# Spijkervet/Context-Aware-Sequential-Recommendation

Hardware: NVIDIA B200
Metric: train_seqs_per_sec (higher is better)
Workload: dtype f32

## Files before the change

### context-aware-sequential-recommendation_b200/_lib.py

```python
from __future__ import annotations

import ctypes as C
import os

_HERE = os.path.dirname(os.path.abspath(__file__))
LIB_PATH = os.path.join(_HERE, "csrc", "libcast_b200.so")

P, L, I, F, U64, SZ = C.c_void_p, C.c_long, C.c_int, C.c_float, C.c_ulonglong, C.c_size_t

SIGNATURES = {
    "cast_version": (I, []),
    "cast_last_error_string": (C.c_char_p, []),
    "cast_launch_count": (U64, []),
    "cast_crc32c": (C.c_uint, [P, SZ, C.c_uint]),
    "cast_embed_fwd": (I, [P, P, I, I, L, I, F, P, P, F, U64, P, I, P, P, P]),
    "cast_mask_dropout": (I, [P, P, F, U64, P, I, L, I, P, P, P]),
    "cast_concat_dropout_fwd": (I, [P, I, I, L, I, F, I, F, I, U64, P, P, P]),
    "cast_concat_dropout_bwd": (I, [P, I, I, L, I, F, I, F, I, U64, P, P, P]),
    "cast_dropout_keep": (I, [F, U64, P, I, L, P, P]),
    "cast_add": (I, [P, P, P, L, P]),
    "cast_relu_bwd": (I, [P, P, F, P, L, P]),
    "cast_layernorm_fwd": (I, [P, P, P, L, I, F, P, P, P, P, P, P]),
    "cast_layernorm_bwd_workspace_bytes": (SZ, [L, I]),
    "cast_layernorm_bwd": (I, [P, P, P, P, P, L, I, P, P, P, P, P, SZ, P]),
    "cast_gemm_set_backend": (I, [I]),
    "cast_gemm_tensor_status": (I, [P, P]),
    "cast_gemm_workspace_bytes": (SZ, [L, I, L, I]),
    "cast_gemm": (I, [P, L, L, P, L, L, P, L, L, I, L, P, I, F, U64, P, I, P, L, F, P, L, P, I, P, SZ, P]),
    "cast_fused_supported": (I, [I]),
    "cast_ln_qkv_fwd": (I, [P, P, P, P, P, P, P, P, P, L, I, F, P, P, P, P, P, P, P, P, P]),
    "cast_ln_ffn_fwd": (I, [P, P, P, P, P, P, P, P, F, U64, P, I, I, L, I, F, P, P, P, P, P, P]),
    "cast_rowk_supported": (I, [I]),
    "cast_rowk_image_bytes": (SZ, [I]),
    "cast_rowk_presplit": (I, [P, I, I, P, SZ, P]),
    "cast_rowk_ln_qkv_fwd": (I, [P, P, P, P, P, P, P, L, I, F, P, P, P, P, P, P, P, P, P]),
    "cast_rowk_ln_ffn_fwd": (I, [P, P, P, P, P, P, P, F, U64, P, I, I, L, I, F, P, P, P, P, P, P]),
    "cast_rowk_status": (I, [P]),
    "cast_rowk_set_grid": (I, [I]),
    "cast_rowk_set_trace": (I, [P]),
    "cast_block_bwd_workspace_bytes": (SZ, [L, I]),
    "cast_ffn_bwd": (I, [P, P, P, P, P, P, P, P, P, P, F, U64, P, I, L, I, P, P, P, SZ, P]),
    "cast_qkv_bwd": (I, [P, P, P, P, P, P, P, P, P, P, P, P, L, I, P, P, P, SZ, P]),
    "cast_qkv_bwd_embed": (I, [P, P, P, P, P, P, P, P, P, P, P, P, L, I, P, F, U64, P, I, P, P, P, SZ, P]),
    "cast_colsum_workspace_bytes": (SZ, [L, L]),
    "cast_colsum": (I, [P, L, L, L, P, P, SZ, P]),
    "cast_attn_set_chunk": (I, [I]),
    "cast_set_pdl": (I, [I]),
    "cast_attn_set_kg": (I, [I]),
    "cast_fused_set_backend": (I, [I]),
    "cast_block_bwd_parts": (I, [L, I]),
    "cast_reduce_partials_batch": (I, [I, P, P, P, P, P, P]),
    "cast_layernorm_bwd_parts": (I, [L]),
    "cast_logits_loss_parts": (I, [L]),
    "cast_sampler_create": (P, [I, I, P, P, P, P, P, P, I, C.c_uint, P, I]),
    "cast_sampler_next": (I, [P, I, P, P, P, P, P, P, P, P]),
    "cast_sampler_next_raw": (I, [P, I, P, P, P, P, P]),
    "cast_sampler_destroy": (None, [P]),
    "cast_time_features": (I, [P, P, P, I, I, P, I, P, P, P, P]),
    "cast_lnf_loss_parts": (I, [L]),
    "cast_lnf_loss_workspace_bytes": (SZ, [L, I]),
    "cast_lnf_loss": (I, [P, P, P, F, P, I, I, L, P, P, P, P, P, P, P, P, P, SZ, P]),
    "cast_attn_fwd": (I, [P, L, P, L, P, L, P, P, P, I, I, I, I, F, U64, P, I, P, P, P, P, P, P]),
    "cast_attn_bwd": (I, [P, L, P, L, P, L, P, P, P, P, P, P, P, I, I, I, I, F, U64, P, I, P, L, P, L, P, L, P, P, P, SZ,
                      P]),
    "cast_attn_bwd_workspace_bytes": (SZ, [I, I, I]),
    "cast_logits_loss_workspace_bytes": (SZ, [L]),
    "cast_logits_loss": (I, [P, P, I, I, L, P, P, P, P, P, P, P, P, P, SZ, P]),
    "cast_scatter_workspace_bytes": (SZ, [L, I, I]),
    "cast_scatter_partial_bytes": (SZ, [L, I, I]),
    "cast_scatter_rows": (I, [P, I, L, P, P, P, I, I, P, P, SZ, P, SZ, P]),
    "cast_scatter_sort": (I, [P, I, L, I, P, SZ, P]),
    "cast_scatter_apply": (I, [I, L, P, P, P, I, I, P, P, SZ, P, SZ, I, P]),
    "cast_adam_init_state": (I, [P, F, F, P]),
    "cast_adam_tf_step": (I, [P, P, P, P, L, F, F, F, F, P, F, L, L, P, P]),
    "cast_adam_tf_range": (I, [P, P, P, P, L, F, F, F, F, P, F, L, L, P, I, P]),
    "cast_adam_tf_step_peers": (I, [P, P, I, P, P, P, L, L, F, F, F, F, F, L, L, P, P]),
    "cast_score_rank_cand": (I, [P, L, P, I, I, L, P, I, P, P, P, P]),
    "cast_score_rank_full_workspace_bytes": (SZ, [L, I, I]),
    "cast_score_rank_full": (I, [P, L, P, I, I, L, P, P, P, P, I, P, P, P, P, SZ, P]),
    "cast_embed_fwd_sharded": (I, [P, P, I, I, I, L, I, F, P, P, F, U64, P, I, P, P, P]),
    "cast_logits_loss_sharded": (I, [P, P, I, I, I, L, P, P, P, P, P, P, P, P, P, SZ, P]),
    "cast_score_rank_cand_sharded": (I, [P, L, P, I, I, I, L, P, I, P, P, P, P]),
    "cast_scatter_set_chunk": (I, [I]),
    "cast_scatter_sort_sharded": (I, [P, I, L, I, I, I, P, SZ, P]),
    "cast_scatter_sorted_offsets": (I, [L, I, I, P, P]),
    "cast_scatter_apply_range": (I, [I, L, P, P, P, I, P, P, P, C.c_uint, C.c_uint, P, SZ, I, P]),
    "cast_scatter_stage_bytes": (SZ, [L, I, I]),
    "cast_scatter_pull_range": (I, [I, L, P, P, P, I, P, P, P, C.c_uint, C.c_uint, P, SZ, P, SZ, I, P]),
    "cast_peer_alloc": (I, [SZ, P, P]),
    "cast_peer_free": (I, [P]),
    "cast_peer_open": (I, [P, P]),
    "cast_peer_close": (I, [P]),
    "cast_peer_barrier": (I, [P, I, I, P, P]),
    "cast_peer_reduce": (I, [P, I, L, P, P]),
    "cast_score_rank_full_status": (I, [P, L, I, P, P]),
    "cast_topk_full_workspace_bytes": (SZ, [L, I, I, I]),
    "cast_topk_full": (I, [P, L, P, I, I, L, I, P, P, I, P, P, P, P, SZ, P]),
    "cast_topk_full_status": (I, [P, L, I, I, I, P, P]),
}


class CastError(RuntimeError):
    pass


def bind(lib: C.CDLL) -> C.CDLL:
    for name, (res, args) in SIGNATURES.items():
        try:
            fn = getattr(lib, name)
        except AttributeError as e:
            raise CastError(f"{name} is not exported by {getattr(lib, '_name', lib)}") from e
        fn.restype = res
        fn.argtypes = args
    return lib


_LIB = None


def load_library(path: str | None = None) -> C.CDLL:
    global _LIB
    if _LIB is not None and path is None:
        return _LIB
    p = path or LIB_PATH
    if not os.path.isfile(p):
        raise CastError(
            f"CUDA extension not found at {p}. Build it with `python -c 'import __graft_entry__ as g; g.build()'` "
            "(nvcc, sm_100a). This package has no CPU / PyTorch fallback.")
    lib = bind(C.CDLL(p))
    if os.environ.get("CAST_ATTN_CHUNK"):
        check(lib, lib.cast_attn_set_chunk(int(os.environ["CAST_ATTN_CHUNK"])), "cast_attn_set_chunk")
    if os.environ.get("CAST_PDL"):
        check(lib, lib.cast_set_pdl(int(os.environ["CAST_PDL"])), "cast_set_pdl")
    if os.environ.get("CAST_ATTN_KG"):
        check(lib, lib.cast_attn_set_kg(int(os.environ["CAST_ATTN_KG"])), "cast_attn_set_kg")
    if os.environ.get("CAST_FUSED_BACKEND"):
        check(lib, lib.cast_fused_set_backend(int(os.environ["CAST_FUSED_BACKEND"])), "cast_fused_set_backend")
    if path is None:
        _LIB = lib
    return lib


def check(lib: C.CDLL, rc: int, what: str = ""):
    if rc != 0:
        msg = lib.cast_last_error_string()
        raise CastError(f"{what} failed with code {rc}: {msg.decode() if msg else ''}")
```

### context-aware-sequential-recommendation_b200/csrc/row_umma.cu

```cuda
#include "cast_rt.cuh"
#include "mma_tf32.cuh"
#include "umma.cuh"

namespace cast {

constexpr int RU_ROWS = 128;
constexpr int RU_ROW_THREADS = 512;
constexpr int RU_THREADS = RU_ROW_THREADS + 32;
constexpr int RU_PA = RU_ROWS * 16 + 16;
constexpr int RU_NIMG = 9;
constexpr size_t RU_SMEM_MAX = 232448;

struct RuShape {
  int H, KS, SL, NP;
  int img1, img2;
  int dense;
};

__host__ __device__ inline RuShape ru_shape(int H) {
  RuShape s;
  s.H = H;
  s.KS = (H + 7) / 8;
  s.SL = 2 * s.KS;
  s.NP = (H + 15) / 16 * 16;
  s.img1 = 2 * s.SL * (s.NP * 16 + 16);
  s.img2 = 2 * s.SL * (2 * s.NP * 16 + 16);
  s.dense = (RU_ROWS * H * 4 + 15) & ~15;
  return s;
}

__host__ __device__ inline size_t ru_img_offset(const RuShape& s, int which) {
  size_t off = 0;
  for (int i = 0; i < which; ++i) off += (i == 1) ? s.img2 : s.img1;
  return off;
}
__host__ __device__ inline size_t ru_img_block_bytes(const RuShape& s) { return ru_img_offset(s, RU_NIMG); }

struct RuPresplitArgs {
  const float* w[16][5];
};

__global__ void __launch_bounds__(256) ru_presplit_kernel(RuPresplitArgs a, int H, unsigned char* __restrict__ images) {
  const RuShape s = ru_shape(H);
  const int blk = blockIdx.z, which = blockIdx.y;
  unsigned char* img = images + (size_t)blk * ru_img_block_bytes(s) + ru_img_offset(s, which);
  const int rows = (which == 1) ? 2 * s.NP : s.NP;
  const int pitch = rows * 16 + 16;
  const int half = s.SL * pitch;
  const int KP = 4 * s.SL;
  const bool transposed = which < 4;
  const int idx = blockIdx.x * (int)blockDim.x + threadIdx.x;
  if (idx >= rows * KP) return;
  int n, k;
  if (transposed) { k = idx / rows; n = idx - k * rows; } else { n = idx / KP; k = idx - n * KP; }
  const float* W;
  int nn = n;
  switch (which) {
    case 0: case 4: W = a.w[blk][0]; break;
    case 1: W = a.w[blk][n < s.NP ? 1 : 2]; nn = n < s.NP ? n : n - s.NP; break;
    case 2: case 7: W = a.w[blk][3]; break;
    case 3: case 8: W = a.w[blk][4]; break;
    case 5: W = a.w[blk][1]; break;
    default: W = a.w[blk][2]; break;
  }
  float v = 0.f;
  if (nn < H && k < H) v = transposed ? W[k * H + nn] : W[nn * H + k];
  unsigned hi, lo;
  tf32_split(v, hi, lo);
  const int off = (k >> 2) * pitch + n * 16 + (k & 3) * 4;
  *reinterpret_cast<unsigned*>(img + off) = hi;
  *reinterpret_cast<unsigned*>(img + half + off) = lo;
}


#ifndef CAST_EMU
__device__ __forceinline__ void ru_cp_async16(float* dst, const float* src, int bytes) {
  const unsigned d = (unsigned)__cvta_generic_to_shared(dst);
  asm volatile("cp.async.cg.shared.global [%0], [%1], 16, %2;" ::"r"(d), "l"(src), "r"(bytes) : "memory");
}
#else
inline void ru_cp_async16(float* dst, const float* src, int bytes) {
  for (int i = 0; i < 4; ++i) dst[i] = (4 * i < bytes) ? src[i] : 0.f;
}
#endif

__device__ __forceinline__ void ru_row_sync() { umma::named_sync(1, RU_ROW_THREADS); }

__device__ __forceinline__ void ru_tile_load_async(float* __restrict__ tile, const float* __restrict__ src, long nvalid,
                                                   int ntotal) {
  const int t = threadIdx.x;
  if ((reinterpret_cast<uintptr_t>(src) & 15) == 0) {
    for (int i = 4 * t; i < ntotal; i += 4 * RU_ROW_THREADS) {
      long left = (nvalid - i) * 4;
      const int bytes = left >= 16 ? 16 : (left > 0 ? (int)left : 0);
      ru_cp_async16(tile + i, bytes > 0 ? src + i : src, bytes);
    }
  } else {
    for (int i = t; i < ntotal; i += RU_ROW_THREADS) tile[i] = i < nvalid ? src[i] : 0.f;
  }
  cp_async_commit();
}

__device__ __forceinline__ void ru_tile_store(float* __restrict__ dst, const float* __restrict__ tile, long nvalid) {
  const int t = threadIdx.x;
  if ((reinterpret_cast<uintptr_t>(dst) & 15) == 0) {
    const int n4 = (int)(nvalid >> 2);
    for (int i = t; i < n4; i += RU_ROW_THREADS)
      reinterpret_cast<float4*>(dst)[i] = reinterpret_cast<const float4*>(tile)[i];
    for (int i = 4 * n4 + t; i < nvalid; i += RU_ROW_THREADS) dst[i] = tile[i];
  } else {
    for (int i = t; i < nvalid; i += RU_ROW_THREADS) dst[i] = tile[i];
  }
}

__device__ __forceinline__ void ru_row_load(const float* __restrict__ tile, int r, int c0, int H, float (&x)[16]) {
  const float* p = tile + r * H + c0;
  if ((H & 1) == 0) {
#pragma unroll
    for (int i = 0; i < 16; i += 2) {
      if (c0 + i < H) {
        const float2 v = *reinterpret_cast<const float2*>(p + i);
        x[i] = v.x;
        x[i + 1] = v.y;
      } else {
        x[i] = x[i + 1] = 0.f;
      }
    }
  } else {
#pragma unroll
    for (int i = 0; i < 16; ++i) x[i] = (c0 + i < H) ? p[i] : 0.f;
  }
}

__device__ __forceinline__ void ru_row_store(float* __restrict__ tile, int r, int c0, int H, const float (&x)[16]) {
  float* p = tile + r * H + c0;
  if ((H & 1) == 0) {
#pragma unroll
    for (int i = 0; i < 16; i += 2)
      if (c0 + i < H) *reinterpret_cast<float2*>(p + i) = make_float2(x[i], x[i + 1]);
  } else {
#pragma unroll
    for (int i = 0; i < 16; ++i)
      if (c0 + i < H) p[i] = x[i];
  }
}

__device__ __forceinline__ void ru_stage(unsigned char* __restrict__ hi, unsigned char* __restrict__ lo, int r, int qd,
                                         int SL, const float (&x)[16]) {
#pragma unroll
  for (int i = 0; i < 4; ++i) {
    const int s = 4 * qd + i;
    if (s < SL) {
      uint4 h, l;
      tf32_split(x[4 * i + 0], h.x, l.x);
      tf32_split(x[4 * i + 1], h.y, l.y);
      tf32_split(x[4 * i + 2], h.z, l.z);
      tf32_split(x[4 * i + 3], h.w, l.w);
      *reinterpret_cast<uint4*>(hi + s * RU_PA + r * 16) = h;
      *reinterpret_cast<uint4*>(lo + s * RU_PA + r * 16) = l;
    }
  }
}

__device__ __forceinline__ void ru_operand_ready(uint64_t* bar) {
  umma::fence_smem_to_async();
  umma::fence_before_sync();
  __syncwarp();
  if ((threadIdx.x & 31) == 0) umma::mbar_arrive(bar);
}

__device__ __forceinline__ void ru_issue(uint32_t tmem_d, uint32_t a_hi, uint32_t a_lo, uint32_t b_hi, uint32_t b_lo,
                                         uint32_t b_pitch, int KS, uint32_t idesc, uint32_t accumulate) {
  uint64_t dah = umma::smem_desc(a_hi, RU_PA, 128), dal = umma::smem_desc(a_lo, RU_PA, 128);
  uint64_t dbh = umma::smem_desc(b_hi, b_pitch, 128), dbl = umma::smem_desc(b_lo, b_pitch, 128);
  for (int ks = 0; ks < KS; ++ks) {
    umma::mma_tf32(tmem_d, dal, dbh, idesc, (ks > 0) ? 1u : accumulate);
    umma::mma_tf32(tmem_d, dah, dbl, idesc, 1u);
    umma::mma_tf32(tmem_d, dah, dbh, idesc, 1u);
    dah = umma::desc_advance(dah, 2 * RU_PA);
    dal = umma::desc_advance(dal, 2 * RU_PA);
    dbh = umma::desc_advance(dbh, 2 * b_pitch);
    dbl = umma::desc_advance(dbl, 2 * b_pitch);
  }
}

__device__ long long* g_rowk_trace = nullptr;
#ifndef CAST_EMU
#define RU_STAMP(slot, k)                                                                      \
  if (trace && threadIdx.x == 0 && (slot) < 4) trace[((long)blockIdx.x * 4 + (slot)) * 16 + (k)] = clock64()
#else
#define RU_STAMP(slot, k)
#endif

__device__ int g_rowk_timeout = 0;
__device__ __forceinline__ void ru_wait(uint64_t* bar, uint32_t parity) {
  if (!umma::mbar_wait(bar, parity, 1u << 22)) g_rowk_timeout = 1;
}

struct RuRange {
  long lo, hi;
  int ntiles;
};
__device__ __forceinline__ RuRange ru_range(long N, long rpc) {
  RuRange g;
  g.lo = (long)blockIdx.x * rpc;
  g.hi = g.lo + rpc < N ? g.lo + rpc : N;
  g.ntiles = g.hi > g.lo ? (int)((g.hi - g.lo + RU_ROWS - 1) / RU_ROWS) : 0;
  return g;
}

struct RuLn {
  float mean, rstd, xsum;
};
template <class F>
__device__ __forceinline__ RuLn ru_layernorm(const float (&x)[16], float (&y)[16], const float* __restrict__ gamma,
                                             const float* __restrict__ beta, float eps, int r, int qd, int c0, int H,
                                             float* __restrict__ red, F&& between) {
  float sp = 0.f;
#pragma unroll
  for (int i = 0; i < 16; ++i) sp += x[i];
  red[r * 4 + qd] = sp;
  ru_row_sync();
  between();
  RuLn o;
  {
    const float4 p = *reinterpret_cast<const float4*>(red + r * 4);
    o.xsum = (p.x + p.y) + (p.z + p.w);
  }
  o.mean = o.xsum / (float)H;
  float qp = 0.f;
#pragma unroll
  for (int i = 0; i < 16; ++i) {
    const float d = (c0 + i < H) ? x[i] - o.mean : 0.f;
    y[i] = d;
    qp += d * d;
  }
  red[512 + r * 4 + qd] = qp;
  ru_row_sync();
  {
    const float4 p = *reinterpret_cast<const float4*>(red + 512 + r * 4);
    o.rstd = 1.0f / sqrtf(((p.x + p.y) + (p.z + p.w)) / (float)H + eps);
  }
  float yp = 0.f;
#pragma unroll
  for (int i = 0; i < 16; i += 4) {
    const float4 g = *reinterpret_cast<const float4*>(gamma + c0 + i);
    const float4 b = *reinterpret_cast<const float4*>(beta + c0 + i);
    y[i + 0] = (c0 + i + 0 < H) ? g.x * (y[i + 0] * o.rstd) + b.x : 0.f;
    y[i + 1] = (c0 + i + 1 < H) ? g.y * (y[i + 1] * o.rstd) + b.y : 0.f;
    y[i + 2] = (c0 + i + 2 < H) ? g.z * (y[i + 2] * o.rstd) + b.z : 0.f;
    y[i + 3] = (c0 + i + 3 < H) ? g.w * (y[i + 3] * o.rstd) + b.w : 0.f;
    yp += (y[i] + y[i + 1]) + (y[i + 2] + y[i + 3]);
  }
  red[1024 + r * 4 + qd] = yp;
  return o;
}

struct RuLnQkvArgs {
  const float *x, *gamma, *beta, *bq, *bk, *bv;
  const unsigned char* img;
  float eps;
  float *qn, *Q, *K, *V, *mean, *rstd, *kmask, *qmask;
  long N, rpc;
  int H;
};

__global__ void __launch_bounds__(RU_THREADS, 1) ru_ln_qkv_fwd_kernel(RuLnQkvArgs a) {
  CAST_DYN_SMEM(unsigned char, sm);
  __shared__ __align__(8) uint64_t bars[5];
  __shared__ uint32_t tmem_slot;
  const RuShape s = ru_shape(a.H);
  const int H = a.H;
  unsigned char* wq = sm;
  unsigned char* wkv = wq + s.img1;
  unsigned char* a_hi = wkv + s.img2;
  unsigned char* a_lo = a_hi + s.SL * RU_PA;
  float* tin = reinterpret_cast<float*>(a_lo + s.SL * RU_PA);
  float* out0 = tin + s.dense / 4;
  float* out1 = out0 + s.dense / 4;
  float* vec = out1 + s.dense / 4;
  float* red = vec + 5 * 64;
  const int t = threadIdx.x, warp = t >> 5, r = t & 127, qd = (t >> 7) & 3, c0 = 16 * qd;
  const bool have_cols = c0 < H;
  long long* trace = g_rowk_trace;
  RU_STAMP(0, 0);

  if (t == 0) {
    umma::mbar_init(&bars[0], 1);
    umma::mbar_init(&bars[1], RU_ROW_THREADS / 32);
    umma::mbar_init(&bars[2], RU_ROW_THREADS / 32);
    umma::mbar_init(&bars[3], 1);
    umma::mbar_init(&bars[4], 1);
  }
  if (warp == 0) umma::tmem_alloc(&tmem_slot, 256);
  for (int i = t; i < 5 * 64; i += RU_THREADS) {
    const int which = i >> 6, c = i & 63;
    const float* src = which == 0 ? a.gamma : which == 1 ? a.beta : which == 2 ? a.bq : which == 3 ? a.bk : a.bv;
    vec[i] = c < H ? src[c] : 0.f;
  }
  umma::fence_before_sync();
  __syncthreads();
  umma::fence_after_sync();
  const uint32_t tmem = tmem_slot;
  const RuRange rg = ru_range(a.N, a.rpc);
  const uint32_t idesc_q = umma::idesc_tf32(128, s.NP), idesc_kv = umma::idesc_tf32(128, 2 * s.NP);

  if (warp == RU_ROW_THREADS / 32) {
    if ((t & 31) == 0 && rg.ntiles > 0) {
      umma::mbar_arrive_expect_tx(&bars[0], (uint32_t)(s.img1 + s.img2));
      umma::bulk_g2s(wq, a.img + ru_img_offset(s, 0), (uint32_t)s.img1, &bars[0]);
      umma::bulk_g2s(wkv, a.img + ru_img_offset(s, 1), (uint32_t)s.img2, &bars[0]);
      cast_pdl_wait();
      ru_wait(&bars[0], 0);
      for (int it = 0; it < rg.ntiles; ++it) {
        const uint32_t par = (uint32_t)(it & 1);
        ru_wait(&bars[1], par);
        umma::fence_after_sync();
        ru_issue(tmem + (uint32_t)s.NP, umma::smem_u32(a_hi), umma::smem_u32(a_lo), umma::smem_u32(wkv),
                 umma::smem_u32(wkv + s.img2 / 2), (uint32_t)(2 * s.NP * 16 + 16), s.KS, idesc_kv, 0u);
        umma::mma_commit(&bars[3]);
        ru_wait(&bars[2], par);
        umma::fence_after_sync();
        ru_issue(tmem, umma::smem_u32(a_hi), umma::smem_u32(a_lo), umma::smem_u32(wq), umma::smem_u32(wq + s.img1 / 2),
                 (uint32_t)(s.NP * 16 + 16), s.KS, idesc_q, 0u);
        umma::mma_commit(&bars[4]);
      }
    }
    __syncwarp();
  } else {
    const int ntot = RU_ROWS * H;
    auto rows_of = [&](int it) {
      const long left = rg.hi - (rg.lo + (long)it * RU_ROWS);
      return left < RU_ROWS ? left : (long)RU_ROWS;
    };
    cast_pdl_wait();
    if (rg.ntiles > 0) ru_tile_load_async(tin, a.x + rg.lo * H, rows_of(0) * H, ntot);
    const uint32_t lane_base = ((uint32_t)(warp & 3) * 32u) << 16;
    for (int it = 0; it < rg.ntiles; ++it) {
      const long row0 = rg.lo + (long)it * RU_ROWS, row = row0 + r;
      const long vrows = rows_of(it), nvalid = vrows * H;
      const uint32_t par = (uint32_t)(it & 1);
      cp_async_wait<0>();
      ru_row_sync();
      RU_STAMP(it, 1);
      float x[16], q[16];
      ru_row_load(tin, r, c0, H, x);
      ru_stage(a_hi, a_lo, r, qd, s.SL, x);
      ru_operand_ready(&bars[1]);
      RU_STAMP(it, 2);
      const RuLn ln = ru_layernorm(x, q, vec, vec + 64, a.eps, r, qd, c0, H, red, [&]() {
        if (it + 1 < rg.ntiles) ru_tile_load_async(tin, a.x + (row0 + RU_ROWS) * H, rows_of(it + 1) * H, ntot);
      });
      RU_STAMP(it, 3);
      ru_row_store(out0, r, c0, H, q);
      ru_wait(&bars[3], par);
      umma::fence_after_sync();
      RU_STAMP(it, 4);
      ru_stage(a_hi, a_lo, r, qd, s.SL, q);
      ru_operand_ready(&bars[2]);
      ru_row_sync();
      RU_STAMP(it, 5);
      if (qd == 0 && row < rg.hi) {
        const float4 p = *reinterpret_cast<const float4*>(red + 1024 + r * 4);
        const float ysum = (p.x + p.y) + (p.z + p.w);
        a.mean[row] = ln.mean;
        a.rstd[row] = ln.rstd;
        if (a.kmask) a.kmask[row] = ln.xsum != 0.f ? 1.f : 0.f;
        if (a.qmask) a.qmask[row] = ysum != 0.f ? 1.f : 0.f;
      }
      ru_tile_store(a.qn + row0 * H, out0, nvalid);
      float v[16];
      if (have_cols) {
        umma::tmem_ld16(tmem + lane_base + (uint32_t)(s.NP + c0), v);
#pragma unroll
        for (int i = 0; i < 16; ++i) v[i] += vec[3 * 64 + c0 + i];
        ru_row_store(out1, r, c0, H, v);
      }
      ru_row_sync();
      RU_STAMP(it, 6);
      ru_tile_store(a.K + row0 * H, out1, nvalid);
      if (have_cols) {
        umma::tmem_ld16(tmem + lane_base + (uint32_t)(2 * s.NP + c0), v);
#pragma unroll
        for (int i = 0; i < 16; ++i) v[i] += vec[4 * 64 + c0 + i];
        ru_row_store(out0, r, c0, H, v);
      }
      ru_row_sync();
      RU_STAMP(it, 7);
      ru_tile_store(a.V + row0 * H, out0, nvalid);
      ru_wait(&bars[4], par);
      umma::fence_after_sync();
      RU_STAMP(it, 8);
      if (have_cols) {
        umma::tmem_ld16(tmem + lane_base + (uint32_t)c0, v);
#pragma unroll
        for (int i = 0; i < 16; ++i) v[i] += vec[2 * 64 + c0 + i];
        ru_row_store(out1, r, c0, H, v);
      }
      umma::fence_before_sync();
      ru_row_sync();
      ru_tile_store(a.Q + row0 * H, out1, nvalid);
      RU_STAMP(it, 9);
    }
    cp_async_wait<0>();
  }
  umma::fence_before_sync();
  __syncthreads();
  if (warp == 0) umma::tmem_free(tmem, 256);
}

struct RuLnFfnArgs {
  const float *y, *gamma, *beta, *b1, *b2;
  const unsigned char* img;
  const int* ids;
  float eps, rate;
  unsigned long long seed;
  const unsigned long long* step;
  int site_h, site_o;
  float *zn, *h1d, *xout, *mean, *rstd;
  long N, rpc;
  int H;
};

__global__ void __launch_bounds__(RU_THREADS, 1) ru_ln_ffn_fwd_kernel(RuLnFfnArgs a) {
  CAST_DYN_SMEM(unsigned char, sm);
  __shared__ __align__(8) uint64_t bars[5];
  __shared__ uint32_t tmem_slot;
  const RuShape s = ru_shape(a.H);
  const int H = a.H;
  unsigned char* w1 = sm;
  unsigned char* w2 = w1 + s.img1;
  unsigned char* a_hi = w2 + s.img1;
  unsigned char* a_lo = a_hi + s.SL * RU_PA;
  float* tin = reinterpret_cast<float*>(a_lo + s.SL * RU_PA);
  float* out0 = tin + s.dense / 4;
  float* out1 = out0 + s.dense / 4;
  float* vec = out1 + s.dense / 4;
  float* red = vec + 4 * 64;
  const int t = threadIdx.x, warp = t >> 5, r = t & 127, qd = (t >> 7) & 3, c0 = 16 * qd;
  const bool have_cols = c0 < H;
  long long* trace = g_rowk_trace;
  RU_STAMP(0, 0);

  if (t == 0) {
    umma::mbar_init(&bars[0], 1);
    umma::mbar_init(&bars[1], RU_ROW_THREADS / 32);
    umma::mbar_init(&bars[2], RU_ROW_THREADS / 32);
    umma::mbar_init(&bars[3], 1);
    umma::mbar_init(&bars[4], 1);
  }
  if (warp == 0) umma::tmem_alloc(&tmem_slot, 128);
  for (int i = t; i < 4 * 64; i += RU_THREADS) {
    const int which = i >> 6, c = i & 63;
    const float* src = which == 0 ? a.gamma : which == 1 ? a.beta : which == 2 ? a.b1 : a.b2;
    vec[i] = c < H ? src[c] : 0.f;
  }
  umma::fence_before_sync();
  __syncthreads();
  umma::fence_after_sync();
  const uint32_t tmem = tmem_slot;
  const RuRange rg = ru_range(a.N, a.rpc);
  const uint32_t idesc = umma::idesc_tf32(128, s.NP);
  const uint32_t wpitch = (uint32_t)(s.NP * 16 + 16);

  if (warp == RU_ROW_THREADS / 32) {
    if ((t & 31) == 0 && rg.ntiles > 0) {
      umma::mbar_arrive_expect_tx(&bars[0], (uint32_t)(2 * s.img1));
      umma::bulk_g2s(w1, a.img + ru_img_offset(s, 2), (uint32_t)(2 * s.img1), &bars[0]);
      cast_pdl_wait();
      ru_wait(&bars[0], 0);
      for (int it = 0; it < rg.ntiles; ++it) {
        const uint32_t par = (uint32_t)(it & 1);
        ru_wait(&bars[1], par);
        umma::fence_after_sync();
        ru_issue(tmem, umma::smem_u32(a_hi), umma::smem_u32(a_lo), umma::smem_u32(w1), umma::smem_u32(w1 + s.img1 / 2),
                 wpitch, s.KS, idesc, 0u);
        umma::mma_commit(&bars[3]);
        ru_wait(&bars[2], par);
        umma::fence_after_sync();
        ru_issue(tmem + (uint32_t)s.NP, umma::smem_u32(a_hi), umma::smem_u32(a_lo), umma::smem_u32(w2),
                 umma::smem_u32(w2 + s.img1 / 2), wpitch, s.KS, idesc, 0u);
        umma::mma_commit(&bars[4]);
      }
    }
    __syncwarp();
  } else {
    const int ntot = RU_ROWS * H;
    auto rows_of = [&](int it) {
      const long left = rg.hi - (rg.lo + (long)it * RU_ROWS);
      return left < RU_ROWS ? left : (long)RU_ROWS;
    };
    cast_pdl_wait();
    if (rg.ntiles > 0) ru_tile_load_async(tin, a.y + rg.lo * H, rows_of(0) * H, ntot);
    const uint32_t lane_base = ((uint32_t)(warp & 3) * 32u) << 16;
    const Drop dh = make_drop(a.rate, a.seed, a.step, a.site_h);
    const Drop dout = make_drop(a.rate, a.seed, a.step, a.site_o);
    for (int it = 0; it < rg.ntiles; ++it) {
      const long row0 = rg.lo + (long)it * RU_ROWS, row = row0 + r;
      const long vrows = rows_of(it), nvalid = vrows * H;
      const uint32_t par = (uint32_t)(it & 1);
      const float m = (row < rg.hi && a.ids) ? (a.ids[row] != 0 ? 1.f : 0.f) : 1.f;
      cp_async_wait<0>();
      ru_row_sync();
      RU_STAMP(it, 1);
      float x[16], zn[16];
      ru_row_load(tin, r, c0, H, x);
      const RuLn ln = ru_layernorm(x, zn, vec, vec + 64, a.eps, r, qd, c0, H, red, [&]() {
        if (it + 1 < rg.ntiles) ru_tile_load_async(tin, a.y + (row0 + RU_ROWS) * H, rows_of(it + 1) * H, ntot);
      });
      RU_STAMP(it, 2);
      ru_stage(a_hi, a_lo, r, qd, s.SL, zn);
      ru_operand_ready(&bars[1]);
      ru_row_store(out0, r, c0, H, zn);
      if (qd == 0 && row < rg.hi) {
        a.mean[row] = ln.mean;
        a.rstd[row] = ln.rstd;
      }
      ru_row_sync();
      RU_STAMP(it, 3);
      ru_tile_store(a.zn + row0 * H, out0, nvalid);
      ru_wait(&bars[3], par);
      umma::fence_after_sync();
      RU_STAMP(it, 4);
      float v[16];
      const unsigned long long fi0 = (unsigned long long)(row * H + c0);
      const bool fi_even = (fi0 & 1ull) == 0ull;
      if (have_cols) {
        umma::tmem_ld16(tmem + lane_base + (uint32_t)c0, v);
        float dm[16];
        if (fi_even) {
#pragma unroll
          for (int i = 0; i < 16; i += 2) drop_mul2_even(dh, fi0 + i, dm[i], dm[i + 1]);
        } else {
#pragma unroll
          for (int i = 0; i < 16; i += 2) drop_mul2(dh, fi0 + i, dm[i], dm[i + 1]);
        }
#pragma unroll
        for (int i = 0; i < 16; ++i) {
          const int c = c0 + i;
          v[i] = (c < H) ? fmaxf(v[i] + vec[2 * 64 + c], 0.f) * dm[i] : 0.f;
        }
        ru_row_store(out1, r, c0, H, v);
      } else {
#pragma unroll
        for (int i = 0; i < 16; ++i) v[i] = 0.f;
      }
      ru_stage(a_hi, a_lo, r, qd, s.SL, v);
      ru_operand_ready(&bars[2]);
      ru_row_sync();
      RU_STAMP(it, 5);
      ru_tile_store(a.h1d + row0 * H, out1, nvalid);
      ru_wait(&bars[4], par);
      umma::fence_after_sync();
      RU_STAMP(it, 6);
      if (have_cols) {
        umma::tmem_ld16(tmem + lane_base + (uint32_t)(s.NP + c0), v);
        float dm[16];
        if (fi_even) {
#pragma unroll
          for (int i = 0; i < 16; i += 2) drop_mul2_even(dout, fi0 + i, dm[i], dm[i + 1]);
        } else {
#pragma unroll
          for (int i = 0; i < 16; i += 2) drop_mul2(dout, fi0 + i, dm[i], dm[i + 1]);
        }
#pragma unroll
        for (int i = 0; i < 16; ++i) v[i] = ((v[i] + vec[3 * 64 + ((c0 + i) & 63)]) * dm[i] + zn[i]) * m;
        ru_row_store(out0, r, c0, H, v);
      }
      umma::fence_before_sync();
      ru_row_sync();
      ru_tile_store(a.xout + row0 * H, out0, nvalid);
      RU_STAMP(it, 7);
    }
    cp_async_wait<0>();
  }
  umma::fence_before_sync();
  __syncthreads();
  if (warp == 0) umma::tmem_free(tmem, 128);
}

static size_t ru_ln_qkv_smem(const RuShape& s) {
  return (size_t)s.img1 + s.img2 + 2 * (size_t)s.SL * RU_PA + 3 * (size_t)s.dense + (5 * 64 + 3 * 512) * sizeof(float);
}
static size_t ru_ln_ffn_smem(const RuShape& s) {
  return 2 * (size_t)s.img1 + 2 * (size_t)s.SL * RU_PA + 3 * (size_t)s.dense + (4 * 64 + 3 * 512) * sizeof(float);
}

constexpr int RU_NUM_SMS = 148;

}

using namespace cast;

#define CAST_RU_SMEM(kernel, bytes)                                                            \
  {                                                                                            \
    static size_t configured = 48 * 1024;                                                      \
    if ((bytes) > configured) {                                                                \
      cudaFuncSetAttribute(kernel, cudaFuncAttributeMaxDynamicSharedMemorySize, (int)(bytes)); \
      configured = (bytes);                                                                    \
    }                                                                                          \
  }

static int g_rowk_max_ctas = RU_NUM_SMS;
extern "C" int cast_rowk_set_grid(int max_ctas) {
  if (max_ctas < 1) return set_error(CAST_ERR_BAD_ARG, "rowk_set_grid");
  g_rowk_max_ctas = max_ctas < RU_NUM_SMS ? max_ctas : RU_NUM_SMS;
  return CAST_OK;
}

extern "C" int cast_rowk_supported(int H) {
  if (H < 8 || H > 64) return 0;
  const RuShape s = ru_shape(H);
  return ru_ln_qkv_smem(s) <= RU_SMEM_MAX && ru_ln_ffn_smem(s) <= RU_SMEM_MAX;
}

extern "C" size_t cast_rowk_image_bytes(int H) {
  if (H <= 0 || H > 64) return 0;
  return ru_img_block_bytes(ru_shape(H));
}

extern "C" int cast_rowk_presplit(const float* const* weights, int nblocks, int H, void* images, size_t image_bytes,
                                  void* stream) {
  if (!weights || !images || nblocks <= 0) return set_error(CAST_ERR_BAD_ARG, "rowk_presplit");
  if (!cast_rowk_supported(H)) return set_error(CAST_ERR_UNSUPPORTED, "rowk_presplit: hidden_units not supported");
  const size_t per = cast_rowk_image_bytes(H);
  if (image_bytes < per * (size_t)nblocks) return set_error(CAST_ERR_WORKSPACE, "rowk_presplit: image buffer too small");
  for (int b0 = 0; b0 < nblocks; b0 += 16) {
    const int nb = nblocks - b0 < 16 ? nblocks - b0 : 16;
    RuPresplitArgs a;
    for (int b = 0; b < 16; ++b)
      for (int j = 0; j < 5; ++j) a.w[b][j] = b < nb ? weights[(size_t)(b0 + b) * 5 + j] : nullptr;
    for (int b = 0; b < nb; ++b)
      for (int j = 0; j < 5; ++j)
        if (!a.w[b][j]) return set_error(CAST_ERR_BAD_ARG, "rowk_presplit: null weight pointer");
    const RuShape s = ru_shape(H);
    CAST_LAUNCH(ru_presplit_kernel, dim3((unsigned)cdiv(2L * s.NP * 4 * s.SL, 256), RU_NIMG, (unsigned)nb), dim3(256), 0,
                (cudaStream_t)stream, a, H, static_cast<unsigned char*>(images) + (size_t)b0 * per);
  }
  return check_launch("rowk_presplit");
}

extern "C" int cast_rowk_ln_qkv_fwd(const float* x, const float* gamma, const float* beta, const float* bq,
                                    const float* bk, const float* bv, const void* images, long N, int H, float eps,
                                    float* qn, float* Q, float* K, float* V, float* mean, float* rstd, float* kmask,
                                    float* qmask, void* stream) {
  if (!x || !gamma || !beta || !bq || !bk || !bv || !images || !qn || !Q || !K || !V || !mean || !rstd || N <= 0)
    return set_error(CAST_ERR_BAD_ARG, "rowk_ln_qkv_fwd");
  if (!cast_rowk_supported(H)) return set_error(CAST_ERR_UNSUPPORTED, "rowk_ln_qkv_fwd: hidden_units not supported");
  const RuShape s = ru_shape(H);
  const long ntiles = cdiv(N, RU_ROWS);
  const int grid = (int)(ntiles < g_rowk_max_ctas ? ntiles : g_rowk_max_ctas);
  const long rpc = cdiv(cdiv(N, grid), 4) * 4;
  RuLnQkvArgs a{x, gamma, beta, bq, bk, bv, static_cast<const unsigned char*>(images), eps, qn, Q, K, V, mean, rstd,
                kmask, qmask, N, rpc, H};
  const size_t smem = ru_ln_qkv_smem(s);
  CAST_RU_SMEM(ru_ln_qkv_fwd_kernel, smem)
  CAST_LAUNCH_DEP(ru_ln_qkv_fwd_kernel, dim3(grid), dim3(RU_THREADS), smem, (cudaStream_t)stream, a);
  return check_launch("rowk_ln_qkv_fwd");
}

extern "C" int cast_rowk_ln_ffn_fwd(const float* y, const float* gamma, const float* beta, const float* b1,
                                    const float* b2, const void* images, const int* ids, float drop_rate,
                                    unsigned long long seed, const unsigned long long* step, int site_hidden,
                                    int site_out, long N, int H, float eps, float* zn, float* h1d, float* xout,
                                    float* mean, float* rstd, void* stream) {
  if (!y || !gamma || !beta || !b1 || !b2 || !images || !zn || !h1d || !xout || !mean || !rstd || N <= 0)
    return set_error(CAST_ERR_BAD_ARG, "rowk_ln_ffn_fwd");
  if (!cast_rowk_supported(H)) return set_error(CAST_ERR_UNSUPPORTED, "rowk_ln_ffn_fwd: hidden_units not supported");
  if (drop_rate < 0.f || drop_rate >= 1.f) return set_error(CAST_ERR_BAD_ARG, "rowk_ln_ffn_fwd: drop_rate");
  const RuShape s = ru_shape(H);
  const long ntiles = cdiv(N, RU_ROWS);
  const int grid = (int)(ntiles < g_rowk_max_ctas ? ntiles : g_rowk_max_ctas);
  const long rpc = cdiv(cdiv(N, grid), 4) * 4;
  RuLnFfnArgs a{y, gamma, beta, b1, b2, static_cast<const unsigned char*>(images), ids, eps, drop_rate, seed, step,
                site_hidden, site_out, zn, h1d, xout, mean, rstd, N, rpc, H};
  const size_t smem = ru_ln_ffn_smem(s);
  CAST_RU_SMEM(ru_ln_ffn_fwd_kernel, smem)
  CAST_LAUNCH_DEP(ru_ln_ffn_fwd_kernel, dim3(grid), dim3(RU_THREADS), smem, (cudaStream_t)stream, a);
  return check_launch("rowk_ln_ffn_fwd");
}

extern "C" int cast_rowk_set_trace(void* device_buffer) {
#ifndef CAST_EMU
  long long* p = static_cast<long long*>(device_buffer);
  if (cudaMemcpyToSymbol(g_rowk_trace, &p, sizeof(p)) != cudaSuccess) return set_error(CAST_ERR_CUDA, "rowk_set_trace");
#endif
  return CAST_OK;
}

extern "C" int cast_rowk_status(int* timed_out) {
  if (!timed_out) return set_error(CAST_ERR_BAD_ARG, "rowk_status");
#ifdef CAST_EMU
  *timed_out = g_rowk_timeout;
  g_rowk_timeout = 0;
#else
  int v = 0, zero = 0;
  if (cudaDeviceSynchronize() != cudaSuccess) return set_error(CAST_ERR_CUDA, "rowk_status: device error");
  cudaMemcpyFromSymbol(&v, g_rowk_timeout, sizeof(int));
  cudaMemcpyToSymbol(g_rowk_timeout, &zero, sizeof(int));
  *timed_out = v;
#endif
  return CAST_OK;
}
```

### context-aware-sequential-recommendation_b200/engine.py

```python
from __future__ import annotations

import ctypes as C
import math
import os
from types import SimpleNamespace
from typing import Dict, List, Optional

import numpy as np
import torch

from . import _lib

TOWER_ID = {"main": 0, "time": 1, "hours": 2, "days": 3}
SITE_EMBED, SITE_CONCAT_A, SITE_CONCAT_B = 9000, 9001, 9002
MODELS = ["cast_1", "cast_2", "cast_3", "cast_4", "cast_5", "cast_6", "cast_7", "cast_8", "cast_9", "sasrec",
          "sasrec_static"]
TABLE_ROWS = {"hours_emb": 25, "days_emb": 8}


def block_site(tower: str, block: int, k: int) -> int:
    return 1000 * TOWER_ID[tower] + 10 * block + k


def sinusoid_table(dim: int, length: int) -> np.ndarray:
    pos = np.arange(length, dtype=np.float64)[:, None]
    i = np.arange(dim, dtype=np.float64)[None, :]
    v = (pos / np.power(10000.0, 2.0 * i / dim)).reshape(-1)
    v[::2] = np.sin(v[::2])
    v[1::2] = np.cos(v[1::2])
    return v.reshape(length, dim).astype(np.float32)


def model_plan(model: str, args) -> SimpleNamespace:
    m = model.lower()
    if m not in MODELS:
        raise ValueError(f"provide model from {MODELS}")
    L, Lc = args.num_blocks, getattr(args, "num_context_blocks", 2)
    p = SimpleNamespace(model=m, towers={}, tables=["item_emb"], learned_pos=m in ("sasrec", "cast_9"))
    if m in ("cast_1", "cast_2", "cast_3", "cast_4", "cast_5", "cast_6"):
        p.towers["time"] = L
        p.tables.append("time_emb")
    if m in ("cast_3", "cast_4", "cast_5", "cast_6", "cast_7", "cast_8", "cast_9"):
        p.tables += ["hours_emb", "days_emb"]
    if m == "cast_8":
        p.towers["hours"] = L
        p.towers["days"] = L
    if m == "cast_9":
        p.towers["hours"] = Lc
        p.towers["days"] = Lc
        p.towers["time"] = Lc
        p.tables.append("time_emb")
    p.towers["main"] = L
    p.embed = {"sasrec": (False, True, True), "sasrec_static": (False, True, True), "cast_1": (True, True, True),
               "cast_2": (False, False, True), "cast_3": (True, False, True), "cast_4": (False, False, True),
               "cast_5": (True, False, False), "cast_6": (False, False, False), "cast_7": (False, False, True),
               "cast_8": (False, False, True), "cast_9": (False, False, False)}[m]
    p.merge = {"cast_2": (["seq", "time"], 2, False, "pre", False),
               "cast_3": (["seq", "hours", "days"], 3, False, "pre", False),
               "cast_4": (["seq", "time", "hours", "days"], 2, True, "pre", False),
               "cast_5": (["seq", "hours", "days"], 3, False, "post", False),
               "cast_6": (["seq", "time", "hours", "days"], 2, True, "post", False),
               "cast_7": (["seq", "hours", "days"], 3, False, "pre", False),
               "cast_8": (["seq", "hours", "days"], 3, False, "pre", False),
               "cast_9": (["seq", "time", "hours", "days"], 4, False, "pre", True)}.get(m)
    p.attn_tower = "time" if m in ("cast_1", "cast_2", "cast_3", "cast_4", "cast_5", "cast_6") else "main"
    return p


def shard_rows(itemnum: int, world: int) -> int:
    return (itemnum + 1 + world - 1) // world + 1


def param_shapes(plan, args, itemnum: int, item_rows: Optional[int] = None):
    H, T = args.hidden_units, args.maxlen
    out = []
    rows = {"item_emb": itemnum + 1, "time_emb": args.max_bins + 1, **TABLE_ROWS}
    for t in plan.tables:
        if t == "item_emb" and item_rows is not None:
            out.append((t, (item_rows, H), rows[t], H))
            continue
        out.append((t, (rows[t], H), rows[t], H))
    if plan.learned_pos:
        out.append(("pos_emb", (T, H), T, H))
    n_tables = len(out)
    for tower, nb in plan.towers.items():
        for i in range(nb):
            pre = f"{tower}.{i}."
            out.append((pre + "ln1.beta", (H,), None, 0.0))
            out.append((pre + "ln1.gamma", (H,), None, 1.0))
            for d in ("q", "k", "v"):
                out.append((pre + d + ".w", (H, H), H, H))
                out.append((pre + d + ".b", (H,), None, 0.0))
            out.append((pre + "ln2.beta", (H,), None, 0.0))
            out.append((pre + "ln2.gamma", (H,), None, 1.0))
            for d in ("ffn1", "ffn2"):
                out.append((pre + d + ".w", (H, H), H, H))
                out.append((pre + d + ".b", (H,), None, 0.0))
        out.append((f"{tower}.lnf.beta", (H,), None, 0.0))
        out.append((f"{tower}.lnf.gamma", (H,), None, 1.0))
    if plan.merge:
        k = len(plan.merge[0]) * H
        out += [("mlp.0.w", (k, k), k, k), ("mlp.0.b", (k,), None, 0.0), ("mlp.1.w", (k, H), k, H),
                ("mlp.1.b", (H,), None, 0.0)]
    return out, n_tables


class Engine:

    def __init__(self, model: str, usernum: int, itemnum: int, args, device=None, lib=None, seed: Optional[int] = None,
                 item_shard: Optional[tuple] = None, alloc=None):
        self.lib = lib if lib is not None else _lib.load_library()
        self.timing = None
        self.use_fused = True
        if device is None:
            if not torch.cuda.is_available():
                raise _lib.CastError("no CUDA device: this package has no CPU fallback")
            device = torch.device("cuda", torch.cuda.current_device())
        self.device = torch.device(device)
        self.args = args
        self.plan = model_plan(model, args)
        self.usernum, self.itemnum = usernum, itemnum
        self.H, self.T, self.h = args.hidden_units, args.maxlen, args.num_heads
        if self.H % self.h:
            raise ValueError("hidden_units must be divisible by num_heads")
        self.rate = float(args.dropout_rate)
        self.lr = float(args.lr)
        self.l2 = float(getattr(args, "l2_emb", 0.0))
        self.seed = int(seed if seed is not None else (getattr(args, "seed", 0) or 0))
        self.beta1, self.beta2, self.eps = 0.9, 0.98, 1e-8
        self.item_shard = tuple(item_shard) if item_shard is not None and item_shard[1] > 1 else None
        self.V_items = itemnum + 1
        self.shard_R = shard_rows(itemnum, self.item_shard[1]) if self.item_shard else None
        self.alloc = alloc
        self.arena = None
        if self.item_shard is not None and alloc is None:
            from . import dist as _dist
            self.arena = _dist.PeerArena(self.lib, self.device)
            self.alloc = self.arena.alloc
        shapes, n_tables = param_shapes(self.plan, args, itemnum, self.shard_R)
        self.shapes = shapes
        total = sum(int(np.prod(s)) for _, s, _, _ in shapes)
        f32 = dict(dtype=torch.float32, device=self.device)
        self.w = self._peer_zeros(total, torch.float32)
        self.gbuf = torch.zeros(total + 4, **f32)
        self.g = self.gbuf[:total]
        self.sums = self.gbuf[total:]
        self.m = torch.zeros(total, **f32)
        self.v = torch.zeros(total, **f32)
        self.P: Dict[str, torch.Tensor] = {}
        self.G: Dict[str, torch.Tensor] = {}
        self.offsets: Dict[str, int] = {}
        off = 0
        for idx, (name, shape, _, _) in enumerate(shapes):
            n = int(np.prod(shape))
            self.P[name] = self.w[off:off + n].view(*shape)
            self.G[name] = self.g[off:off + n].view(*shape)
            self.offsets[name] = off
            off += n
            if idx == n_tables - 1:
                self.l2_hi = off
        self.n_params = total
        self.adam_state = torch.zeros(2, dtype=torch.int64, device=self.device)
        self.step_ptr = self.adam_state.data_ptr() + 8
        self.sinus = torch.from_numpy(sinusoid_table(self.H, self.T)).to(self.device)
        self.init_parameters(self.seed or 42)
        self._call(self.lib.cast_adam_init_state, self.adam_state.data_ptr(), self.beta1, self.beta2, self._stream())
        self._ctx: Dict[tuple, SimpleNamespace] = {}
        self.use_rowk = bool(self.lib.cast_rowk_supported(self.H))
        self.rowk_block: Dict[str, int] = {}
        if self.use_rowk:
            names = [f"{tower}.{i}." for tower, nb in self.plan.towers.items() for i in range(nb)]
            self.rowk_block = {n: j for j, n in enumerate(names)}
            self.rowk_img_bytes = int(self.lib.cast_rowk_image_bytes(self.H))
            self.rowk_img = torch.zeros(max(1, len(names)) * self.rowk_img_bytes, dtype=torch.uint8, device=self.device)
            ptrs = [self.P[n + w].data_ptr() for n in names for w in ("q.w", "k.w", "v.w", "ffn1.w", "ffn2.w")]
            self.rowk_wptrs = (C.c_void_p * len(ptrs))(*ptrs)
        self.world_size = 1
        self.grad_allreduce = None
        self.adam_g = self.gbuf
        self.exchange_capturable = False
        self.after_adam = None
        if self.device.type == "cuda":
            self.lib.cast_set_pdl(0 if os.environ.get("CAST_PDL", "1") == "0" else 1)
        self.fork_reduce = os.environ.get("CAST_FORK_REDUCE", "1") != "0"
        self.fuse_embed_bwd = os.environ.get("CAST_FUSE_EMBED_BWD", "1") != "0"
        self.before_backward = None
        self.peer_adam = None
        self.shard_ptrs = None

    def _peer_zeros(self, numel, dtype):
        if self.alloc is not None and self.item_shard is not None:
            t = self.alloc(int(numel), dtype)
            t.zero_()
            return t
        return torch.zeros(int(numel), dtype=dtype, device=self.device)

    def _stream(self):
        if self.device.type == "cuda":
            return torch.cuda.current_stream(self.device).cuda_stream
        return None

    def _call(self, fn, *a):
        if self.timing is not None:
            e0, e1 = torch.cuda.Event(enable_timing=True), torch.cuda.Event(enable_timing=True)
            e0.record()
            rc = fn(*a)
            e1.record()
            self.timing.append((fn.__name__, a, e0, e1))
        else:
            rc = fn(*a)
        if rc != 0:
            _lib.check(self.lib, rc, fn.__name__)

    @staticmethod
    def _p(t):
        return None if t is None else t.data_ptr()

    def init_parameters(self, seed: int):
        gen = torch.Generator().manual_seed(seed)
        for name, shape, fan_in, fan_out in self.shapes:
            if fan_in is None:
                self.P[name].fill_(float(fan_out))
            else:
                limit = math.sqrt(6.0 / (fan_in + fan_out))
                if name == "item_emb" and self.item_shard is not None:
                    full = (torch.rand((self.V_items, shape[1]), generator=gen, dtype=torch.float64) * 2 - 1)
                    self.P[name].copy_(self.shard_of(full.mul(limit).float()).to(self.device))
                    continue
                vals = (torch.rand(shape, generator=gen, dtype=torch.float64) * 2 - 1).mul(limit).float()
                self.P[name].copy_(vals.to(self.device))
        self.m.zero_()
        self.v.zero_()

    def shard_of(self, full: torch.Tensor) -> torch.Tensor:
        rank, world = self.item_shard
        out = torch.zeros((self.shard_R,) + tuple(full.shape[1:]), dtype=full.dtype)
        mine = full[rank::world]
        off = 1 if rank else 0
        out[off:off + mine.shape[0]] = mine
        return out

    def rebind_gradients(self, gbuf: torch.Tensor):
        assert gbuf.numel() == self.gbuf.numel()
        local = self.adam_g is self.gbuf
        self.gbuf = gbuf
        self.g = gbuf[:self.n_params]
        self.sums = gbuf[self.n_params:]
        for name, shape, _, _ in self.shapes:
            off = self.offsets[name]
            self.G[name] = self.g[off:off + int(np.prod(shape))].view(*shape)
        if local:
            self.adam_g = gbuf
        for c in self._ctx.values():
            c.sums = self.sums

    def global_sums(self) -> torch.Tensor:
        return self.adam_g[self.n_params:]

    def load_parameters(self, params: Dict[str, "torch.Tensor | np.ndarray"]):
        for k, v in params.items():
            v = torch.as_tensor(np.asarray(v) if not torch.is_tensor(v) else v)
            if k == "item_emb" and self.item_shard is not None and v.shape[0] == self.V_items:
                v = self.shard_of(v)
            self.P[k].copy_(v.to(self.device))

    def state_step(self) -> int:
        return int(self.adam_state[1].item())

    def ctx(self, B: int) -> SimpleNamespace:
        key = (B, bool(self.use_fused))
        c = self._ctx.get(key)
        if c is not None:
            return c
        H, T, h, dev = self.H, self.T, self.h, self.device
        N = B * T
        lib = self.lib
        f = lambda *s: torch.empty(*s, dtype=torch.float32, device=dev)
        fp = (lambda *s: self._peer_zeros(int(np.prod(s)), torch.float32).view(*s)) if self.item_shard else f
        c = SimpleNamespace(B=B, N=N)
        c.keys3 = torch.zeros(3, N, dtype=torch.int32, device=dev)
        c.cids = torch.zeros(3, N, dtype=torch.int32, device=dev)
        c.tw = {}
        for tower, nb in self.plan.towers.items():
            blocks = []
            for _ in range(nb):
                b = SimpleNamespace()
                for nm in ("qn", "Q", "K", "V", "y", "zn", "h1d", "xout"):
                    setattr(b, nm, f(N, H))
                for nm in ("mu1", "rs1", "kmask", "qmask", "mu2", "rs2"):
                    setattr(b, nm, f(N))
                for nm in ("rmax", "rlinv", "rowD"):
                    setattr(b, nm, f(B * h * T))
                if self.use_fused and bool(self.lib.cast_fused_supported(H)):
                    nws = self.lib.cast_block_bwd_workspace_bytes(N, H) // 4 + 16
                    b.ws_ffn, b.ws_qkv = f(nws), f(nws)
                blocks.append(b)
            c.tw[tower] = SimpleNamespace(blocks=blocks, out=(fp if tower == "main" else f)(N, H), muf=f(N), rsf=f(N),
                                          dx_in=f(N, H), x_in=None)
        c.attn_ws = None
        if H // h <= 64 and 2 * B * h * T * T * 4 <= (2 << 30):
            c.attn_ws = torch.empty(self.lib.cast_attn_bwd_workspace_bytes(B, T, h) // 4, dtype=torch.float32, device=dev)
        c.x0 = f(N, H)
        c.emb = {t: f(N, H) for t in self.plan.tables if t != "item_emb"}
        c.demb = {t: f(N, H) for t in self.plan.tables if t != "item_emb"}
        if self.plan.merge:
            k = len(self.plan.merge[0])
            c.cat, c.mlp_h, c.mlp_out = f(N, k * H), f(N, k * H), fp(N, H)
            c.dcat, c.dmlp_h, c.dmlp_o = f(N, k * H), f(N, k * H), f(N, H)
            c.dsrc = {s: f(N, H) for s in self.plan.merge[0]}
        c.pos_logits, c.neg_logits, c.gpos, c.gneg = f(N), f(N), fp(N), fp(N)
        c.sums = self.sums
        c.dseq = f(N, H)
        c.t = [f(N, H) for _ in range(7)]
        c.g0 = fp(N, H)
        kmax = (len(self.plan.merge[0]) if self.plan.merge else 1) * H
        c.splits = int(max(1, min(296, N // 128)))
        ws = max(lib.cast_layernorm_bwd_workspace_bytes(N, H),
                 lib.cast_gemm_workspace_bytes(kmax, kmax, N, c.splits), lib.cast_gemm_workspace_bytes(N, kmax, kmax, 1),
                 lib.cast_colsum_workspace_bytes(N, kmax), lib.cast_colsum_workspace_bytes(B, T * H),
                 lib.cast_logits_loss_workspace_bytes(N), lib.cast_block_bwd_workspace_bytes(N, H))
        c.ws = torch.empty(ws // 4 + 16, dtype=torch.float32, device=dev)
        c.ws_bytes = ws
        vmax = max(self.P[t].shape[0] for t in self.plan.tables)
        if self.item_shard:
            vmax = max(vmax, self.item_shard[1] * self.shard_R)
        sws = lib.cast_scatter_workspace_bytes(N, 3, vmax)
        c.sws = self._peer_zeros(sws // 4 + 16, torch.int32) if self.item_shard else \
            torch.empty(sws // 4 + 16, dtype=torch.int32, device=dev)
        c.sws_bytes = sws
        c.peer = None
        spb = lib.cast_scatter_partial_bytes(N, 3, H)
        c.spart = torch.empty(spb // 4 + 16, dtype=torch.float32, device=dev)
        c.spart_bytes = spb
        c.attn = None
        c.graph = None
        self._ctx[key] = c
        return c

    def _gemm(self, A, sam, sak, Bm, sbk, sbn, Cm, ldc, M, N, K, c, bias=None, relu=0, rate=0.0, site=0, act=None,
              ld_act=0, act_scale=1.0, resid=None, ldr=0, row_ids=None, splits=1):
        self._call(self.lib.cast_gemm, A.data_ptr(), sam, sak, Bm.data_ptr(), sbk, sbn, Cm.data_ptr(), ldc, M, N, K,
                   self._p(bias), relu, rate, self.seed, self.step_ptr, site, self._p(act), ld_act, act_scale,
                   self._p(resid), ldr, self._p(row_ids), splits, c.ws.data_ptr(), c.ws_bytes, self._stream())

    def linear_fwd(self, c, X, W, b, Y, **kw):
        N, K = X.shape
        M = W.shape[1]
        self._gemm(X, K, 1, W, M, 1, Y, M, N, M, K, c, bias=b, **kw)

    def linear_dgrad(self, c, dY, W, dX, **kw):
        N, M = dY.shape
        K = W.shape[0]
        self._gemm(dY, M, 1, W, 1, M, dX, K, N, K, M, c, **kw)

    def linear_wgrad(self, c, X, dY, dW, db):
        N, K = X.shape
        M = dY.shape[1]
        self._gemm(X, 1, K, dY, M, 1, dW, M, K, M, N, c, splits=c.splits)
        if db is not None:
            self._call(self.lib.cast_colsum, dY.data_ptr(), N, M, M, db.data_ptr(), c.ws.data_ptr(), c.ws_bytes,
                       self._stream())

    def ln_fwd(self, x, pre, y, mu, rs, xnz=None, ynz=None):
        N = x.shape[0]
        self._call(self.lib.cast_layernorm_fwd, x.data_ptr(), self.P[pre + ".gamma"].data_ptr(),
                   self.P[pre + ".beta"].data_ptr(), N, self.H, 1e-8, y.data_ptr(), self._p(mu), self._p(rs),
                   self._p(xnz), self._p(ynz), self._stream())

    def ln_bwd(self, c, dy, x, mu, rs, pre, dx, dx_add=None):
        N = x.shape[0]
        self._call(self.lib.cast_layernorm_bwd, dy.data_ptr(), x.data_ptr(), mu.data_ptr(), rs.data_ptr(),
                   self.P[pre + ".gamma"].data_ptr(), N, self.H, self._p(dx_add), dx.data_ptr(),
                   self.G[pre + ".gamma"].data_ptr(), self.G[pre + ".beta"].data_ptr(), c.ws.data_ptr(), c.ws_bytes,
                   self._stream())

    def embed_fwd(self, ids, table, out, pos=None, add=None, rate=0.0, site=0, mask_ids=None):
        N = ids.numel()
        if self.item_shard is not None and table is self.P["item_emb"]:
            self._call(self.lib.cast_embed_fwd_sharded, ids.data_ptr(), self.shard_ptrs.data_ptr(), self.item_shard[1],
                       self.V_items, self.H, N, self.T, float(self.H ** 0.5), self._p(pos), self._p(add), rate,
                       self.seed, self.step_ptr, site, self._p(mask_ids), out.data_ptr(), self._stream())
            return
        self._call(self.lib.cast_embed_fwd, ids.data_ptr(), table.data_ptr(), table.shape[0], self.H, N, self.T,
                   float(self.H ** 0.5), self._p(pos), self._p(add), rate, self.seed, self.step_ptr, site,
                   self._p(mask_ids), out.data_ptr(), self._stream())

    def mask_dropout(self, x, ids, rate, site, out_m, out_md):
        N = x.shape[0]
        self._call(self.lib.cast_mask_dropout, x.data_ptr(), self._p(ids), rate, self.seed, self.step_ptr, site, N,
                   x.shape[1], self._p(out_m), self._p(out_md), self._stream())

    def scatter(self, c, keys, nsrc, rows, rowscale, scale, table_name):
        N = c.N
        V = self.P[table_name].shape[0]
        rows_a = (C.c_void_p * nsrc)(*[r.data_ptr() for r in rows])
        rs_a = (C.c_void_p * nsrc)(*[(r.data_ptr() if r is not None else None) for r in rowscale])
        sc_a = (C.c_float * nsrc)(*scale)
        if table_name == "item_emb" and self.item_shard is not None:
            if getattr(c, "presorted", False):
                torch.cuda.current_stream(self.device).wait_stream(c.side)
                c.presorted = False
            else:
                self._call(self.lib.cast_scatter_sort_sharded, keys.data_ptr(), nsrc, N, self.V_items,
                           self.item_shard[1], self.shard_R, c.sws.data_ptr(), c.sws_bytes, self._stream())
            if rows[0] is not c.g0:
                c.g0.copy_(rows[0])
            c.shard_src = (nsrc, [c.g0] + list(rows[1:]), list(rowscale), list(scale))
            return
        if table_name == "item_emb" and getattr(c, "presorted", False):
            torch.cuda.current_stream(self.device).wait_stream(c.side)
            c.presorted = False
            self._call(self.lib.cast_scatter_apply, nsrc, N, rows_a, rs_a, sc_a, V, self.H,
                       self.G[table_name].data_ptr(), c.sws.data_ptr(), c.sws_bytes, c.spart.data_ptr(),
                       c.spart_bytes, 0, self._stream())
            return
        self._call(self.lib.cast_scatter_rows, keys.data_ptr(), nsrc, N, rows_a, rs_a, sc_a, V, self.H,
                   self.G[table_name].data_ptr(), c.sws.data_ptr(), c.sws_bytes, c.spart.data_ptr(), c.spart_bytes,
                   self._stream())

    def tower_fwd(self, c, tower, x_in, ids, train, want_attn=False):
        tb = c.tw[tower]
        tb.x_in = x_in
        rate = self.rate if train else 0.0
        H, B, T, h = self.H, c.B, self.T, self.h
        x = x_in
        nb = len(tb.blocks)
        fused = self.use_fused and bool(self.lib.cast_fused_supported(H))
        rowk = self.rowk_active()
        if rowk and getattr(c, "presplit_pending", False):
            torch.cuda.current_stream(self.device).wait_stream(c.side2)
            c.presplit_pending = False
        P = self.P
        for i, b in enumerate(tb.blocks):
            pre = f"{tower}.{i}."
            if rowk:
                self._call(self.lib.cast_rowk_ln_qkv_fwd, x.data_ptr(), P[pre + "ln1.gamma"].data_ptr(),
                           P[pre + "ln1.beta"].data_ptr(), P[pre + "q.b"].data_ptr(), P[pre + "k.b"].data_ptr(),
                           P[pre + "v.b"].data_ptr(), self.rowk_image(pre), c.N, H, 1e-8, b.qn.data_ptr(),
                           b.Q.data_ptr(), b.K.data_ptr(), b.V.data_ptr(), b.mu1.data_ptr(), b.rs1.data_ptr(),
                           b.kmask.data_ptr(), b.qmask.data_ptr(), self._stream())
            elif fused:
                self._call(self.lib.cast_ln_qkv_fwd, x.data_ptr(), P[pre + "ln1.gamma"].data_ptr(),
                           P[pre + "ln1.beta"].data_ptr(), P[pre + "q.w"].data_ptr(), P[pre + "q.b"].data_ptr(),
                           P[pre + "k.w"].data_ptr(), P[pre + "k.b"].data_ptr(), P[pre + "v.w"].data_ptr(),
                           P[pre + "v.b"].data_ptr(), c.N, H, 1e-8, b.qn.data_ptr(), b.Q.data_ptr(), b.K.data_ptr(),
                           b.V.data_ptr(), b.mu1.data_ptr(), b.rs1.data_ptr(), b.kmask.data_ptr(),
                           b.qmask.data_ptr(), self._stream())
            else:
                self.ln_fwd(x, pre + "ln1", b.qn, b.mu1, b.rs1, b.kmask, b.qmask)
                self.linear_fwd(c, b.qn, self.P[pre + "q.w"], self.P[pre + "q.b"], b.Q)
                self.linear_fwd(c, x, self.P[pre + "k.w"], self.P[pre + "k.b"], b.K)
                self.linear_fwd(c, x, self.P[pre + "v.w"], self.P[pre + "v.b"], b.V)
            attn = None
            if want_attn and i == nb - 1:
                if c.attn is None or c.attn.shape[0] != h * B:
                    c.attn = torch.empty(h * B, T, T, dtype=torch.float32, device=self.device)
                attn = c.attn
            self._call(self.lib.cast_attn_fwd, b.Q.data_ptr(), H, b.K.data_ptr(), H, b.V.data_ptr(), H,
                       b.qn.data_ptr(), b.kmask.data_ptr(), b.qmask.data_ptr(), B, T, H, h, rate, self.seed,
                       self.step_ptr, block_site(tower, i, 1), ids.data_ptr(), b.y.data_ptr(), self._p(attn),
                       b.rmax.data_ptr(), b.rlinv.data_ptr(), self._stream())
            if rowk:
                self._call(self.lib.cast_rowk_ln_ffn_fwd, b.y.data_ptr(), P[pre + "ln2.gamma"].data_ptr(),
                           P[pre + "ln2.beta"].data_ptr(), P[pre + "ffn1.b"].data_ptr(), P[pre + "ffn2.b"].data_ptr(),
                           self.rowk_image(pre), ids.data_ptr(), rate, self.seed, self.step_ptr,
                           block_site(tower, i, 2), block_site(tower, i, 3), c.N, H, 1e-8, b.zn.data_ptr(),
                           b.h1d.data_ptr(), b.xout.data_ptr(), b.mu2.data_ptr(), b.rs2.data_ptr(), self._stream())
            elif fused:
                self._call(self.lib.cast_ln_ffn_fwd, b.y.data_ptr(), P[pre + "ln2.gamma"].data_ptr(),
                           P[pre + "ln2.beta"].data_ptr(), P[pre + "ffn1.w"].data_ptr(), P[pre + "ffn1.b"].data_ptr(),
                           P[pre + "ffn2.w"].data_ptr(), P[pre + "ffn2.b"].data_ptr(), ids.data_ptr(), rate,
                           self.seed, self.step_ptr, block_site(tower, i, 2), block_site(tower, i, 3), c.N, H, 1e-8,
                           b.zn.data_ptr(), b.h1d.data_ptr(), b.xout.data_ptr(), b.mu2.data_ptr(), b.rs2.data_ptr(),
                           self._stream())
            else:
                self.ln_fwd(b.y, pre + "ln2", b.zn, b.mu2, b.rs2)
                self.linear_fwd(c, b.zn, self.P[pre + "ffn1.w"], self.P[pre + "ffn1.b"], b.h1d, relu=1, rate=rate,
                                site=block_site(tower, i, 2))
                self.linear_fwd(c, b.h1d, self.P[pre + "ffn2.w"], self.P[pre + "ffn2.b"], b.xout, rate=rate,
                                site=block_site(tower, i, 3), resid=b.zn, ldr=H, row_ids=ids)
            x = b.xout
        if tower == "main" and train and getattr(c, "fuse_tail", False):
            tb.x_last = x
            return tb.out
        self.ln_fwd(x, tower + ".lnf", tb.out, tb.muf, tb.rsf)
        return tb.out

    def tower_bwd(self, c, tower, d_out, ids, embed_fx=None):
        tb = c.tw[tower]
        H, B, T, h = self.H, c.B, self.T, self.h
        rate = self.rate
        scale = 1.0 / (1.0 - rate) if rate > 0 else 1.0
        t = c.t
        nb = len(tb.blocks)
        x_last = tb.blocks[-1].xout if nb else tb.x_in
        fused = self.use_fused and bool(self.lib.cast_fused_supported(H))
        dx = t[0]
        if tower == "main" and getattr(c, "fuse_tail", False):
            pass
        elif fused:
            if getattr(tb, "ws_lnf", None) is None:
                nb_ = self.lib.cast_layernorm_bwd_workspace_bytes(c.N, H)
                tb.ws_lnf = torch.empty(nb_ // 4 + 16, dtype=torch.float32, device=self.device)
            self._call(self.lib.cast_layernorm_bwd, d_out.data_ptr(), x_last.data_ptr(), tb.muf.data_ptr(),
                       tb.rsf.data_ptr(), self.P[tower + ".lnf.gamma"].data_ptr(), c.N, H, None, dx.data_ptr(), None,
                       None, tb.ws_lnf.data_ptr(), tb.ws_lnf.numel() * 4, self._stream())
            parts = self.lib.cast_layernorm_bwd_parts(c.N)
            c.reduce_jobs.append((tb.ws_lnf.data_ptr(), parts, H, self.G[tower + ".lnf.gamma"], 2 * H))
            c.reduce_jobs.append((tb.ws_lnf.data_ptr() + 4 * H, parts, H, self.G[tower + ".lnf.beta"], 2 * H))
        else:
            self.ln_bwd(c, d_out, x_last, tb.muf, tb.rsf, tower + ".lnf", dx)
        for i in reversed(range(nb)):
            b = tb.blocks[i]
            pre = f"{tower}.{i}."
            x_i = tb.blocks[i - 1].xout if i > 0 else tb.x_in
            gm, gmd, dh, dzn, dy = t[1], t[2], t[3], t[4], t[5]
            if fused:
                P = self.P
                self._call(self.lib.cast_ffn_bwd, dx.data_ptr(), ids.data_ptr(), b.zn.data_ptr(), b.h1d.data_ptr(),
                           b.y.data_ptr(), b.mu2.data_ptr(), b.rs2.data_ptr(), P[pre + "ln2.gamma"].data_ptr(),
                           P[pre + "ffn1.w"].data_ptr(), P[pre + "ffn2.w"].data_ptr(), rate, self.seed, self.step_ptr,
                           block_site(tower, i, 3), c.N, H, dy.data_ptr(), None,
                           b.ws_ffn.data_ptr(), b.ws_ffn.numel() * 4, self._stream())
                cnt = 2 * H + 2 * (H * H + H)
                c.reduce_jobs.append((b.ws_ffn.data_ptr(), self.lib.cast_block_bwd_parts(c.N, 0), cnt,
                                      self.G[pre + "ln2.beta"], cnt))
                dQ, dK, dV = t[1], t[2], t[3]
                self._call(self.lib.cast_attn_bwd, b.Q.data_ptr(), H, b.K.data_ptr(), H, b.V.data_ptr(), H,
                           dy.data_ptr(), b.kmask.data_ptr(), b.qmask.data_ptr(), b.rmax.data_ptr(),
                           b.rlinv.data_ptr(), ids.data_ptr(), b.rowD.data_ptr(), B, T, H, h, rate, self.seed,
                           self.step_ptr,
                           block_site(tower, i, 1), dQ.data_ptr(), H, dK.data_ptr(), H, dV.data_ptr(), H,
                           b.y.data_ptr(), b.qn.data_ptr(), self._p(c.attn_ws),
                           c.attn_ws.numel() * 4 if c.attn_ws is not None else 0, self._stream())
                dst = tb.dx_in if i == 0 else t[0]
                if i == 0 and embed_fx is not None:
                    fx_ids, fx_rate, fx_site, dst = embed_fx
                    self._call(self.lib.cast_qkv_bwd_embed, dQ.data_ptr(), dK.data_ptr(), dV.data_ptr(),
                               dy.data_ptr(), x_i.data_ptr(), b.qn.data_ptr(), b.mu1.data_ptr(), b.rs1.data_ptr(),
                               P[pre + "ln1.gamma"].data_ptr(), P[pre + "q.w"].data_ptr(), P[pre + "k.w"].data_ptr(),
                               P[pre + "v.w"].data_ptr(), c.N, H, self._p(fx_ids), float(fx_rate), self.seed,
                               self.step_ptr, int(fx_site), dst.data_ptr(), None, b.ws_qkv.data_ptr(),
                               b.ws_qkv.numel() * 4, self._stream())
                else:
                    self._call(self.lib.cast_qkv_bwd, dQ.data_ptr(), dK.data_ptr(), dV.data_ptr(), dy.data_ptr(),
                               x_i.data_ptr(), b.qn.data_ptr(), b.mu1.data_ptr(), b.rs1.data_ptr(),
                               P[pre + "ln1.gamma"].data_ptr(), P[pre + "q.w"].data_ptr(), P[pre + "k.w"].data_ptr(),
                               P[pre + "v.w"].data_ptr(), c.N, H, dst.data_ptr(), None,
                               b.ws_qkv.data_ptr(), b.ws_qkv.numel() * 4, self._stream())
                cnt = 2 * H + 3 * (H * H + H)
                c.reduce_jobs.append((b.ws_qkv.data_ptr(), self.lib.cast_block_bwd_parts(c.N, 1), cnt,
                                      self.G[pre + "ln1.beta"], cnt))
                dx = dst
                continue
            self.mask_dropout(dx, ids, rate, block_site(tower, i, 3), gm, gmd)
            self.linear_wgrad(c, b.h1d, gmd, self.G[pre + "ffn2.w"], self.G[pre + "ffn2.b"])
            self.linear_dgrad(c, gmd, self.P[pre + "ffn2.w"], dh, act=b.h1d, ld_act=H, act_scale=scale)
            self.linear_wgrad(c, b.zn, dh, self.G[pre + "ffn1.w"], self.G[pre + "ffn1.b"])
            self.linear_dgrad(c, dh, self.P[pre + "ffn1.w"], dzn, resid=gm, ldr=H)
            self.ln_bwd(c, dzn, b.y, b.mu2, b.rs2, pre + "ln2", dy)
            dQ, dK, dV = t[1], t[2], t[3]
            self._call(self.lib.cast_attn_bwd, b.Q.data_ptr(), H, b.K.data_ptr(), H, b.V.data_ptr(), H,
                       dy.data_ptr(), b.kmask.data_ptr(), b.qmask.data_ptr(), b.rmax.data_ptr(), b.rlinv.data_ptr(),
                       ids.data_ptr(), b.rowD.data_ptr(), B, T, H, h, rate, self.seed, self.step_ptr,
                       block_site(tower, i, 1),
                       dQ.data_ptr(), H, dK.data_ptr(), H, dV.data_ptr(), H, b.y.data_ptr(), b.qn.data_ptr(),
                       self._p(c.attn_ws), c.attn_ws.numel() * 4 if c.attn_ws is not None else 0, self._stream())
            self.linear_wgrad(c, b.qn, dQ, self.G[pre + "q.w"], self.G[pre + "q.b"])
            self.linear_wgrad(c, x_i, dK, self.G[pre + "k.w"], self.G[pre + "k.b"])
            self.linear_wgrad(c, x_i, dV, self.G[pre + "v.w"], self.G[pre + "v.b"])
            dqn, dxk, dxkv = t[4], t[6], t[0]
            self.linear_dgrad(c, dQ, self.P[pre + "q.w"], dqn, resid=dy, ldr=H)
            self.linear_dgrad(c, dK, self.P[pre + "k.w"], dxk)
            self.linear_dgrad(c, dV, self.P[pre + "v.w"], dxkv, resid=dxk, ldr=H)
            dst = tb.dx_in if i == 0 else t[5]
            self.ln_bwd(c, dqn, x_i, b.mu1, b.rs1, pre + "ln1", dst, dx_add=dxkv)
            dx = dst
        if nb == 0:
            tb.dx_in.copy_(dx)
        return tb.dx_in

    def merge_fwd(self, c, srcs: Dict[str, torch.Tensor], ids, train):
        names, wa, second, _, mask_after = self.plan.merge
        k = len(names)
        rate = self.rate if train else 0.0
        ptrs = (C.c_void_p * k)(*[srcs[n].data_ptr() for n in names])
        if second:
            ra, sa, rb, sb = rate, SITE_CONCAT_A, rate, SITE_CONCAT_B
        else:
            wa, ra, sa, rb, sb = 0, 0.0, SITE_CONCAT_A, rate, SITE_CONCAT_A
        self._call(self.lib.cast_concat_dropout_fwd, ptrs, k, wa, c.N, self.H, ra, sa, rb, sb, self.seed,
                   self.step_ptr, c.cat.data_ptr(), self._stream())
        self.linear_fwd(c, c.cat, self.P["mlp.0.w"], self.P["mlp.0.b"], c.mlp_h, relu=1)
        self.linear_fwd(c, c.mlp_h, self.P["mlp.1.w"], self.P["mlp.1.b"], c.mlp_out, relu=1,
                        row_ids=ids if mask_after else None)
        return c.mlp_out

    def merge_bwd(self, c, d_out):
        names, wa, second, _, _ = self.plan.merge
        k = len(names)
        rate = self.rate
        n1 = c.N * self.H
        self._call(self.lib.cast_relu_bwd, d_out.data_ptr(), c.mlp_out.data_ptr(), 1.0, c.dmlp_o.data_ptr(), n1,
                   self._stream())
        self.linear_wgrad(c, c.mlp_h, c.dmlp_o, self.G["mlp.1.w"], self.G["mlp.1.b"])
        self.linear_dgrad(c, c.dmlp_o, self.P["mlp.1.w"], c.dmlp_h, act=c.mlp_h, ld_act=k * self.H, act_scale=1.0)
        self.linear_wgrad(c, c.cat, c.dmlp_h, self.G["mlp.0.w"], self.G["mlp.0.b"])
        self.linear_dgrad(c, c.dmlp_h, self.P["mlp.0.w"], c.dcat)
        ptrs = (C.c_void_p * k)(*[c.dsrc[n].data_ptr() for n in names])
        if second:
            ra, sa, rb, sb = rate, SITE_CONCAT_A, rate, SITE_CONCAT_B
        else:
            wa, ra, sa, rb, sb = 0, 0.0, SITE_CONCAT_A, rate, SITE_CONCAT_A
        self._call(self.lib.cast_concat_dropout_bwd, c.dcat.data_ptr(), k, wa, c.N, self.H, ra, sa, rb, sb, self.seed,
                   self.step_ptr, ptrs, self._stream())
        return c.dsrc

    def rowk_active(self):
        return self.use_rowk and self.use_fused and bool(self.rowk_block)

    def rowk_presplit(self, stream):
        self._call(self.lib.cast_rowk_presplit, self.rowk_wptrs, len(self.rowk_block), self.H,
                   self.rowk_img.data_ptr(), self.rowk_img.numel(), stream)

    def rowk_image(self, pre: str) -> int:
        return self.rowk_img.data_ptr() + self.rowk_block[pre] * self.rowk_img_bytes

    def forward(self, c, train: bool, want_attn: bool = False):
        plan = self.plan
        ids = c.keys3[0]
        if self.rowk_active() and not getattr(c, "presplit_pending", False):
            self.rowk_presplit(self._stream())
        streams: Dict[str, torch.Tensor] = {}
        for j, (tname, key) in enumerate((("time_emb", "time"), ("hours_emb", "hours"), ("days_emb", "days"))):
            if tname in plan.tables:
                self.embed_fwd(c.cids[j], self.P[tname], c.emb[tname])
                s = c.emb[tname]
                if key in plan.towers:
                    s = self.tower_fwd(c, key, s, ids, train, want_attn and plan.attn_tower == key)
                streams[key] = s
        add_time, drop, mask = plan.embed
        pos = self.P["pos_emb"] if plan.learned_pos else self.sinus
        self.embed_fwd(ids, self.P["item_emb"], c.x0, pos=pos, add=streams["time"] if add_time else None,
                       rate=self.rate if (train and drop) else 0.0, site=SITE_EMBED, mask_ids=ids if mask else None)
        x = c.x0
        if plan.merge and plan.merge[3] == "pre":
            x = self.merge_fwd(c, {"seq": x, **streams}, ids, train)
        x = self.tower_fwd(c, "main", x, ids, train, want_attn and plan.attn_tower == "main")
        if plan.merge and plan.merge[3] == "post":
            x = self.merge_fwd(c, {"seq": x, **streams}, ids, train)
        c.seq_emb = x
        return x

    def tail_fusable(self):
        plan = self.plan
        return (self.use_fused and bool(self.lib.cast_fused_supported(self.H)) and self.item_shard is None
                and not (plan.merge and plan.merge[3] == "post"))

    def loss_tail_fused(self, c):
        tb = c.tw["main"]
        H, N = self.H, c.N
        if getattr(c, "ws_tail", None) is None:
            c.ws_tail = torch.empty(self.lib.cast_lnf_loss_workspace_bytes(N, H) // 4 + 16, dtype=torch.float32,
                                    device=self.device)
        parts = self.lib.cast_lnf_loss_parts(N)
        self._call(self.lib.cast_lnf_loss, tb.x_last.data_ptr(), self.P["main.lnf.gamma"].data_ptr(),
                   self.P["main.lnf.beta"].data_ptr(), 1e-8, self.P["item_emb"].data_ptr(),
                   self.P["item_emb"].shape[0], H, N, c.keys3[1].data_ptr(), c.keys3[2].data_ptr(), tb.out.data_ptr(),
                   c.pos_logits.data_ptr(), c.neg_logits.data_ptr(), c.gpos.data_ptr(), c.gneg.data_ptr(),
                   c.t[0].data_ptr(), c.ws_tail.data_ptr(), c.ws_tail.numel() * 4, self._stream())
        base = c.ws_tail.data_ptr()
        c.reduce_jobs.append((base, parts, 3, c.sums, 3))
        c.reduce_jobs.append((base + 4 * 3 * parts, parts, H, self.G["main.lnf.gamma"], 2 * H))
        c.reduce_jobs.append((base + 4 * (3 * parts + H), parts, H, self.G["main.lnf.beta"], 2 * H))

    def loss_fwd_bwd(self, c, with_grad=True, defer_sums=False):
        ws, ws_bytes, sums = c.ws, c.ws_bytes, c.sums
        if defer_sums:
            if getattr(c, "ws_loss", None) is None:
                c.ws_loss = torch.empty(self.lib.cast_logits_loss_workspace_bytes(c.N) // 4 + 16, dtype=torch.float32,
                                        device=self.device)
            ws, ws_bytes, sums = c.ws_loss, c.ws_loss.numel() * 4, None
            c.reduce_jobs.append((c.ws_loss.data_ptr(), self.lib.cast_logits_loss_parts(c.N), 3, c.sums, 3))
        tail = (c.keys3[1].data_ptr(), c.keys3[2].data_ptr(), c.pos_logits.data_ptr(), c.neg_logits.data_ptr(),
                self._p(sums), c.dseq.data_ptr() if with_grad else None, c.gpos.data_ptr() if with_grad else None,
                c.gneg.data_ptr() if with_grad else None, ws.data_ptr(), ws_bytes, self._stream())
        if self.item_shard is not None:
            self._call(self.lib.cast_logits_loss_sharded, c.seq_emb.data_ptr(), self.shard_ptrs.data_ptr(),
                       self.item_shard[1], self.V_items, self.H, c.N, *tail)
        else:
            self._call(self.lib.cast_logits_loss, c.seq_emb.data_ptr(), self.P["item_emb"].data_ptr(),
                       self.P["item_emb"].shape[0], self.H, c.N, *tail)

    def backward(self, c):
        plan = self.plan
        ids = c.keys3[0]
        d = c.dseq
        if getattr(c, "reduce_jobs", None) is None:
            c.reduce_jobs = []
        dstreams: Dict[str, torch.Tensor] = {}
        if plan.merge and plan.merge[3] == "post":
            ds = self.merge_bwd(c, d)
            d = ds["seq"]
            dstreams.update({k: v for k, v in ds.items() if k != "seq"})
        add_time, drop, mask = plan.embed
        pre_merge = bool(plan.merge and plan.merge[3] == "pre")
        fuse_embed = ((drop or mask) and not pre_merge and self.use_fused and self.fuse_embed_bwd
                      and len(c.tw["main"].blocks) > 0
                      and bool(self.lib.cast_fused_supported(self.H)))
        d = self.tower_bwd(c, "main", d, ids, embed_fx=(ids if mask else None, self.rate if drop else 0.0, SITE_EMBED,
                                                        c.g0) if fuse_embed else None)
        if pre_merge:
            if plan.merge[4]:
                pass
            ds = self.merge_bwd(c, d)
            d = ds["seq"]
            dstreams.update({k: v for k, v in ds.items() if k != "seq"})
        g0 = d
        if fuse_embed:
            g0 = c.g0
        elif drop or mask:
            self.mask_dropout(d, ids if mask else None, self.rate if drop else 0.0, SITE_EMBED, None, c.g0)
            g0 = c.g0
        if add_time:
            dstreams["time"] = g0
        if plan.learned_pos:
            th = self.T * self.H
            if self.use_fused and bool(self.lib.cast_fused_supported(self.H)):
                c.reduce_jobs.append((g0.data_ptr(), c.B, th, self.G["pos_emb"], th))
            else:
                self._call(self.lib.cast_colsum, g0.data_ptr(), c.B, th, th, self.G["pos_emb"].data_ptr(),
                           c.ws.data_ptr(), c.ws_bytes, self._stream())
        sq = float(self.H ** 0.5)
        ctx_scatter = []
        for j, (tname, key) in enumerate((("time_emb", "time"), ("hours_emb", "hours"), ("days_emb", "days"))):
            if tname not in plan.tables:
                continue
            dk = dstreams[key]
            if key in plan.towers:
                dk = self.tower_bwd(c, key, dk, ids)
            ctx_scatter.append((j, dk, tname))
        forked = self.fork_reduce and self.device.type == "cuda" and self.timing is None and bool(c.reduce_jobs)
        if forked:
            main = torch.cuda.current_stream(self.device)
            if getattr(c, "side3", None) is None:
                c.side3 = torch.cuda.Stream(device=self.device)
            c.side3.wait_stream(main)
            with torch.cuda.stream(c.side3):
                self.flush_reduce_jobs(c)
        try:
            self.scatter(c, c.keys3, 3, [g0, c.seq_emb, c.seq_emb], [None, c.gpos, c.gneg], [sq, 1.0, 1.0], "item_emb")
            for j, dk, tname in ctx_scatter:
                self.scatter(c, c.cids[j], 1, [dk], [None], [sq], tname)
        finally:
            if forked:
                torch.cuda.current_stream(self.device).wait_stream(c.side3)
        self.flush_reduce_jobs(c)

    def rank_local(self):
        import contextlib

        @contextlib.contextmanager
        def cm():
            saved = (self.grad_allreduce, self.after_adam, self.before_backward, self.peer_adam)
            self.grad_allreduce = self.after_adam = self.before_backward = self.peer_adam = None
            try:
                yield self
            finally:
                self.grad_allreduce, self.after_adam, self.before_backward, self.peer_adam = saved
        return cm()

    def flush_reduce_jobs(self, c):
        jobs = c.reduce_jobs
        if not jobs:
            return
        import ctypes as C
        n = len(jobs)
        parts = (C.c_void_p * n)(*[int(j[0]) for j in jobs])
        nparts = (C.c_int * n)(*[int(j[1]) for j in jobs])
        counts = (C.c_long * n)(*[int(j[2]) for j in jobs])
        pitches = (C.c_long * n)(*[int(j[4]) for j in jobs])
        outs = (C.c_void_p * n)(*[j[3].data_ptr() for j in jobs])
        self._call(self.lib.cast_reduce_partials_batch, n, parts, nparts, counts, pitches, outs, self._stream())
        c.reduce_jobs = []

    def adam(self, c):
        if self.peer_adam is not None:
            ptrs, n_ranks, g_red = self.peer_adam
            self._call(self.lib.cast_adam_tf_step_peers, self.w.data_ptr(), ptrs.data_ptr(), n_ranks, g_red.data_ptr(),
                       self.m.data_ptr(), self.v.data_ptr(), self.n_params, g_red.numel() - self.n_params, self.lr,
                       self.beta1, self.beta2, self.eps, self.l2, 0, self.l2_hi if self.l2 else 0,
                       self.adam_state.data_ptr(), self._stream())
            return
        self._call(self.lib.cast_adam_tf_step, self.w.data_ptr(), self.adam_g.data_ptr(), self.m.data_ptr(),
                   self.v.data_ptr(), self.n_params, self.lr, self.beta1, self.beta2, self.eps,
                   self.adam_g[self.n_params + 2:].data_ptr(), self.l2, 0, self.l2_hi if self.l2 else 0,
                   self.adam_state.data_ptr(), self._stream())

    def launch_fwd_bwd(self, c):
        c.presorted = False
        if self.device.type == "cuda" and self.timing is None:
            main = torch.cuda.current_stream(self.device)
            if getattr(c, "side", None) is None:
                c.side = torch.cuda.Stream(device=self.device)
            c.side.wait_stream(main)
            with torch.cuda.stream(c.side):
                if self.item_shard is not None:
                    self._call(self.lib.cast_scatter_sort_sharded, c.keys3.data_ptr(), 3, c.N, self.V_items,
                               self.item_shard[1], self.shard_R, c.sws.data_ptr(), c.sws_bytes, c.side.cuda_stream)
                else:
                    V = self.P["item_emb"].shape[0]
                    self._call(self.lib.cast_scatter_sort, c.keys3.data_ptr(), 3, c.N, V, c.sws.data_ptr(),
                               c.sws_bytes, c.side.cuda_stream)
            c.presorted = True
            if self.rowk_active():
                if getattr(c, "side2", None) is None:
                    c.side2 = torch.cuda.Stream(device=self.device)
                c.side2.wait_stream(main)
                with torch.cuda.stream(c.side2):
                    self.rowk_presplit(c.side2.cuda_stream)
                c.presplit_pending = True
        c.reduce_jobs = []
        c.fuse_tail = self.tail_fusable()
        bb_forked = False
        if self.before_backward is not None and self.device.type == "cuda" and self.timing is None:
            main = torch.cuda.current_stream(self.device)
            if getattr(c, "side4", None) is None:
                c.side4 = torch.cuda.Stream(device=self.device)
            c.side4.wait_stream(main)
            with torch.cuda.stream(c.side4):
                self.before_backward()
            bb_forked = True
        try:
            try:
                self.forward(c, train=True)
            finally:
                if bb_forked:
                    torch.cuda.current_stream(self.device).wait_stream(c.side4)
            if self.before_backward is not None and not bb_forked:
                self.before_backward()
            if c.fuse_tail:
                self.loss_tail_fused(c)
            else:
                self.loss_fwd_bwd(c, with_grad=True, defer_sums=True)
            self.backward(c)
        finally:
            c.fuse_tail = False
            if getattr(c, "presorted", False) or getattr(c, "presplit_pending", False):
                main = torch.cuda.current_stream(self.device)
                if getattr(c, "presorted", False):
                    main.wait_stream(c.side)
                if getattr(c, "presplit_pending", False):
                    main.wait_stream(c.side2)
                c.presorted = c.presplit_pending = False
            c.reduce_jobs = []

    def launch_train_step(self, c):
        self.launch_fwd_bwd(c)
        if self.grad_allreduce is not None:
            self.grad_allreduce(c)
        self.adam(c)
        if self.after_adam is not None:
            self.after_adam()
```

### include/cast_b200.h

```cpp
#ifndef CAST_B200_H_
#define CAST_B200_H_

#include <stddef.h>
#include <stdint.h>

#ifdef __cplusplus
extern "C" {
#endif

#define CAST_OK 0
#define CAST_ERR_BAD_ARG (-1)
#define CAST_ERR_UNSUPPORTED (-2)
#define CAST_ERR_WORKSPACE (-3)
#define CAST_ERR_CUDA (-4)

#define CAST_ABI_VERSION 1

int cast_version(void);
const char* cast_last_error_string(void);
unsigned long long cast_launch_count(void);
unsigned int cast_crc32c(const void* data, size_t n, unsigned int crc_in);

int cast_embed_fwd(const int* ids, const float* table, int V, int H, long N, int T, float scale, const float* pos,
                   const float* add, float drop_rate, unsigned long long seed, const unsigned long long* step,
                   int site, const int* mask_ids, float* out, void* stream);

int cast_embed_fwd_sharded(const int* ids, const float* const* shards, int nshards, int V, int H, long N, int T,
                           float scale, const float* pos, const float* add, float drop_rate, unsigned long long seed,
                           const unsigned long long* step, int site, const int* mask_ids, float* out, void* stream);
int cast_logits_loss_sharded(const float* seq_emb, const float* const* shards, int nshards, int V, int H, long N,
                             const int* pos, const int* neg, float* pos_logits, float* neg_logits, float* sums,
                             float* dseq, float* gpos, float* gneg, void* workspace, size_t workspace_bytes,
                             void* stream);
int cast_score_rank_cand_sharded(const float* seq_last, long ld, const float* const* shards, int nshards, int V, int H,
                                 long U, const int* cand, int C, float* logits, int* count_greater, int* count_equal,
                                 void* stream);
int cast_scatter_set_chunk(int entries);
int cast_scatter_sort_sharded(const int* keys, int nsrc, long N, int V, int nshards, int rows_per_shard,
                              void* workspace, size_t workspace_bytes, void* stream);
int cast_scatter_sorted_offsets(long N, int nsrc, int Vkeys, size_t* keys_offset, size_t* payload_offset);
int cast_scatter_apply_range(int nsrc, long N, const float* const* rows, const float* const* rowscale,
                             const float* scale, int H, float* dtable, const void* sorted_keys,
                             const void* sorted_payload, unsigned key_lo, unsigned key_hi, void* partial,
                             size_t partial_bytes, int accumulate, void* stream);
size_t cast_scatter_stage_bytes(long N, int nsrc, int H);
int cast_scatter_pull_range(int nsrc, long N, const float* const* rows, const float* const* rowscale,
                            const float* scale, int H, float* dtable, const void* sorted_keys,
                            const void* sorted_payload, unsigned key_lo, unsigned key_hi, void* stage,
                            size_t stage_bytes, void* partial, size_t partial_bytes, int accumulate, void* stream);
int cast_peer_alloc(size_t bytes, void** ptr, void* ipc_handle64);
int cast_peer_free(void* ptr);
int cast_peer_open(const void* ipc_handle64, void** base_ptr);
int cast_peer_close(void* base_ptr);
int cast_peer_barrier(void* const* flags, int rank, int n, void* state, void* stream);
int cast_peer_reduce(const void* const* grads, int n, long count, float* out, void* stream);

int cast_mask_dropout(const float* in, const int* mask_ids, float drop_rate, unsigned long long seed,
                      const unsigned long long* step, int site, long N, int H, float* out_masked,
                      float* out_masked_dropped, void* stream);

int cast_concat_dropout_fwd(const float* const* srcs, int k, int width_a, long N, int H, float rate_a, int site_a,
                            float rate_b, int site_b, unsigned long long seed, const unsigned long long* step,
                            float* cat, void* stream);
int cast_concat_dropout_bwd(const float* dcat, int k, int width_a, long N, int H, float rate_a, int site_a,
                            float rate_b, int site_b, unsigned long long seed, const unsigned long long* step,
                            float* const* dsts, void* stream);

int cast_dropout_keep(float drop_rate, unsigned long long seed, const unsigned long long* step, int site, long n,
                      unsigned char* keep, void* stream);

int cast_add(const float* a, const float* b, float* out, long n, void* stream);
int cast_relu_bwd(const float* dy, const float* act, float scale, float* out, long n, void* stream);

int cast_layernorm_fwd(const float* x, const float* gamma, const float* beta, long N, int H, float eps, float* y,
                       float* mean, float* rstd, float* xnz, float* ynz, void* stream);
size_t cast_layernorm_bwd_workspace_bytes(long N, int H);
int cast_layernorm_bwd(const float* dy, const float* x, const float* mean, const float* rstd, const float* gamma,
                       long N, int H, const float* dx_add, float* dx, float* dgamma, float* dbeta, void* workspace,
                       size_t workspace_bytes, void* stream);

int cast_gemm_set_backend(int which);
int cast_gemm_tensor_status(int* host_flag, void* stream);
size_t cast_gemm_workspace_bytes(long M, int N, long K, int splits);
int cast_gemm(const float* A, long sam, long sak, const float* B, long sbk, long sbn, float* C, long ldc, long M,
              int N, long K, const float* bias, int relu, float drop_rate, unsigned long long seed,
              const unsigned long long* step, int site, const float* act, long ld_act, float act_scale,
              const float* resid, long ldr, const int* row_ids, int splits, void* workspace, size_t workspace_bytes,
              void* stream);

int cast_fused_supported(int H);
int cast_ln_qkv_fwd(const float* x, const float* gamma, const float* beta, const float* Wq, const float* bq,
                    const float* Wk, const float* bk, const float* Wv, const float* bv, long N, int H, float eps,
                    float* qn, float* Q, float* K, float* V, float* mean, float* rstd, float* kmask, float* qmask,
                    void* stream);
int cast_ln_ffn_fwd(const float* y, const float* gamma, const float* beta, const float* W1, const float* b1,
                    const float* W2, const float* b2, const int* ids, float drop_rate, unsigned long long seed,
                    const unsigned long long* step, int site_hidden, int site_out, long N, int H, float eps, float* zn,
                    float* h1d, float* xout, float* mean, float* rstd, void* stream);
int cast_rowk_supported(int H);
size_t cast_rowk_image_bytes(int H);
int cast_rowk_presplit(const float* const* weights, int nblocks, int H, void* images, size_t image_bytes, void* stream);
int cast_rowk_ln_qkv_fwd(const float* x, const float* gamma, const float* beta, const float* bq, const float* bk,
                         const float* bv, const void* images, long N, int H, float eps, float* qn, float* Q, float* K,
                         float* V, float* mean, float* rstd, float* kmask, float* qmask, void* stream);
int cast_rowk_ln_ffn_fwd(const float* y, const float* gamma, const float* beta, const float* b1, const float* b2,
                         const void* images, const int* ids, float drop_rate, unsigned long long seed,
                         const unsigned long long* step, int site_hidden, int site_out, long N, int H, float eps,
                         float* zn, float* h1d, float* xout, float* mean, float* rstd, void* stream);
int cast_rowk_status(int* timed_out);
int cast_rowk_set_grid(int max_ctas);
int cast_rowk_set_trace(void* device_buffer);
int cast_fused_set_backend(int backend);
size_t cast_block_bwd_workspace_bytes(long N, int H);
int cast_block_bwd_parts(long N, int which);
int cast_reduce_partials_batch(int njobs, const float* const* partials, const int* nparts, const long* counts,
                               const long* pitches, float* const* outs, void* stream);
int cast_layernorm_bwd_parts(long N);
int cast_ffn_bwd(const float* dx, const int* ids, const float* zn, const float* h1d, const float* y, const float* mean,
                 const float* rstd, const float* gamma, const float* W1, const float* W2, float drop_rate,
                 unsigned long long seed, const unsigned long long* step, int site_out, long N, int H, float* dy,
                 float* grads_out, void* workspace, size_t workspace_bytes, void* stream);
int cast_qkv_bwd(const float* dQ, const float* dK, const float* dV, const float* dres, const float* x, const float* qn,
                 const float* mean, const float* rstd, const float* gamma, const float* Wq, const float* Wk,
                 const float* Wv, long N, int H, float* dx, float* grads_out, void* workspace, size_t workspace_bytes,
                 void* stream);
int cast_qkv_bwd_embed(const float* dQ, const float* dK, const float* dV, const float* dres, const float* x,
                       const float* qn, const float* mean, const float* rstd, const float* gamma, const float* Wq,
                       const float* Wk, const float* Wv, long N, int H, const int* mask_ids, float drop_rate,
                       unsigned long long seed, const unsigned long long* step, int site, float* dx, float* grads_out,
                       void* workspace, size_t workspace_bytes, void* stream);

size_t cast_colsum_workspace_bytes(long rows, long cols);
int cast_colsum(const float* X, long rows, long cols, long ld, float* out, void* workspace, size_t workspace_bytes,
                void* stream);

int cast_attn_fwd(const float* Q, long ldq, const float* K, long ldk, const float* V, long ldv, const float* queries,
                  const float* kmask, const float* qmask, int B, int T, int H, int h, float drop_rate,
                  unsigned long long seed, const unsigned long long* step, int site, const int* skip_ids, float* out,
                  float* attn_weights, float* row_max, float* row_linv, void* stream);
int cast_set_pdl(int on);
int cast_attn_set_chunk(int columns);
int cast_attn_set_kg(int key_groups);
size_t cast_attn_bwd_workspace_bytes(int B, int T, int h);
int cast_attn_bwd(const float* Q, long ldq, const float* K, long ldk, const float* V, long ldv, const float* dO,
                  const float* kmask, const float* qmask, const float* row_max, const float* row_linv,
                  const int* skip_ids, float* rowD, int B, int T, int H, int h, float drop_rate,
                  unsigned long long seed, const unsigned long long* step, int site, float* dQ, long lddq, float* dK,
                  long lddk, float* dV, long lddv, const float* out, const float* queries, void* workspace,
                  size_t workspace_bytes, void* stream);

void* cast_sampler_create(int usernum, int itemnum, const long* user_ptr, const int* items, const int* ratings,
                          const int* hours, const int* days, const long long* ts, int maxlen, unsigned seed,
                          const long long* edges, int n_edges);
int cast_sampler_next(void* sampler, int B, int* user, int* seq, int* pos, int* neg, int* timeseq, int* ratings,
                      int* hours, int* days);
int cast_sampler_next_raw(void* sampler, int B, int* user, int* seq, int* pos, int* neg, long long* ts);
void cast_sampler_destroy(void* sampler);

int cast_time_features(const long long* ts, const long long* ref, const int* ids, int B, int T, const long long* edges,
                       int n_edges, int* bins, int* hours, int* days, void* stream);

size_t cast_logits_loss_workspace_bytes(long N);
int cast_logits_loss(const float* seq_emb, const float* table, int V, int H, long N, const int* pos, const int* neg,
                     float* pos_logits, float* neg_logits, float* sums, float* dseq, float* gpos, float* gneg,
                     void* workspace, size_t workspace_bytes, void* stream);
int cast_logits_loss_parts(long N);
int cast_lnf_loss_parts(long N);
size_t cast_lnf_loss_workspace_bytes(long N, int H);
int cast_lnf_loss(const float* x, const float* gamma, const float* beta, float eps, const float* table, int V, int H,
                  long N, const int* pos, const int* neg, float* seq_emb, float* pos_logits, float* neg_logits,
                  float* gpos, float* gneg, float* dx, void* workspace, size_t workspace_bytes, void* stream);

size_t cast_scatter_workspace_bytes(long N, int nsrc, int V);
size_t cast_scatter_partial_bytes(long N, int nsrc, int H);
int cast_scatter_sort(const int* keys, int nsrc, long N, int V, void* workspace, size_t workspace_bytes, void* stream);
int cast_scatter_apply(int nsrc, long N, const float* const* rows, const float* const* rowscale, const float* scale,
                       int V, int H, float* dtable, void* workspace, size_t workspace_bytes, void* partial,
                       size_t partial_bytes, int accumulate, void* stream);
int cast_scatter_rows(const int* keys , int nsrc, long N, const float* const* rows,
                      const float* const* rowscale, const float* scale, int V, int H, float* dtable,
                      void* workspace, size_t workspace_bytes, void* partial, size_t partial_bytes, void* stream);

int cast_adam_init_state(void* state , float beta1, float beta2, void* stream);
int cast_adam_tf_step(float* w, const float* grad, float* m, float* v, long n, float lr, float beta1, float beta2,
                      float eps, const float* gdenom, float l2, long l2_lo, long l2_hi, void* state, void* stream);
int cast_adam_tf_range(float* w, const float* grad, float* m, float* v, long n, float lr, float beta1, float beta2,
                       float eps, const float* gdenom, float l2, long l2_lo, long l2_hi, void* state, int advance,
                       void* stream);

int cast_adam_tf_step_peers(float* w, const void* const* grads, int n_ranks, float* g_red, float* m, float* v, long n,
                            long tail, float lr, float beta1, float beta2, float eps, float l2, long l2_lo, long l2_hi,
                            void* state, void* stream);

int cast_score_rank_cand(const float* seq_last, long ld, const float* table, int V, int H, long U, const int* cand,
                         int C, float* logits, int* count_greater, int* count_equal, void* stream);

size_t cast_score_rank_full_workspace_bytes(long U, int V, int H);
int cast_score_rank_full(const float* seq_last, long ld, const float* table, int V, int H, long U, const int* target,
                         const float* target_score, const int* rated_ptr, const int* rated_idx, int mode,
                         int* count_greater, int* count_equal, unsigned long long* stats, void* workspace,
                         size_t workspace_bytes, void* stream);
int cast_score_rank_full_status(const void* workspace, long U, int V, int* host_flag, void* stream);

size_t cast_topk_full_workspace_bytes(long U, int V, int H, int K);
int cast_topk_full(const float* seq_last, long ld, const float* table, int V, int H, long U, int K,
                   const int* excl_ptr, const int* excl_idx, int mode, int* top_ids, float* top_scores,
                   unsigned long long* stats, void* workspace, size_t workspace_bytes, void* stream);
int cast_topk_full_status(const void* workspace, long U, int V, int H, int K, int* host_flag, void* stream);

#ifdef __cplusplus
}
#endif
#endif
```

Baseline: 252,600.

## Skip left-padding rows in row-kernel LN+QKV and LN+FFN forward passes

Adds a per-batch row-map kernel that finds the first non-pad position of each sequence and builds a compacted schedule of 4-row groups. The fused LN+QKV and LN+FFN forward kernels then do their GEMM work only on live groups, gathering and scattering rows through the map. Skipped padded rows get their analytically known constant outputs written directly. This removes tensor-core and memory work on left-padded positions, at the cost of an extra small single-CTA launch, indirect addressing, and assumptions about padded-row values that must hold exactly.

```diff
diff --git a/context-aware-sequential-recommendation_b200/_lib.py b/context-aware-sequential-recommendation_b200/_lib.py
--- a/context-aware-sequential-recommendation_b200/_lib.py
+++ b/context-aware-sequential-recommendation_b200/_lib.py
@@ -35,6 +35,9 @@
     "cast_rowk_presplit": (I, [P, I, I, P, SZ, P]),
     "cast_rowk_ln_qkv_fwd": (I, [P, P, P, P, P, P, P, L, I, F, P, P, P, P, P, P, P, P, P]),
     "cast_rowk_ln_ffn_fwd": (I, [P, P, P, P, P, P, P, F, U64, P, I, I, L, I, F, P, P, P, P, P, P]),
+    "cast_row_map": (I, [P, I, I, P, P]),
+    "cast_rowk_ln_qkv_fwd_sched": (I, [P, P, P, P, P, P, P, L, I, F, P, P, P, P, P, P, P, P, P, P]),
+    "cast_rowk_ln_ffn_fwd_sched": (I, [P, P, P, P, P, P, P, F, U64, P, I, I, L, I, F, P, P, P, P, P, P, P]),
     "cast_rowk_status": (I, [P]),
     "cast_rowk_set_grid": (I, [I]),
     "cast_rowk_set_trace": (I, [P]),
diff --git a/context-aware-sequential-recommendation_b200/csrc/row_umma.cu b/context-aware-sequential-recommendation_b200/csrc/row_umma.cu
--- a/context-aware-sequential-recommendation_b200/csrc/row_umma.cu
+++ b/context-aware-sequential-recommendation_b200/csrc/row_umma.cu
@@ -1,6 +1,8 @@
 #include "cast_rt.cuh"
 #include "mma_tf32.cuh"
 #include "umma.cuh"
+
+#include <initializer_list>
 
 namespace cast {
 
@@ -209,6 +211,123 @@
   return g;
 }
 
+__global__ void __launch_bounds__(1024) ru_row_map_kernel(const int* __restrict__ ids, int B, int T, int* __restrict__ sched) {
+  CAST_DYN_SMEM(int, sm);
+  int* sb = sm;
+  int* live0 = sm + B;
+  int* skip0 = live0 + B;
+  const int t = threadIdx.x, lane = t & 31, warp = t >> 5, nw = (int)blockDim.x >> 5;
+  for (int b = t; b < B; b += blockDim.x) sb[b] = T;
+  __syncthreads();
+  const long N = (long)B * T;
+  for (long i = t; i < N; i += blockDim.x)
+    if (ids[i] != 0) atomicMin(&sb[i / T], (int)(i % T));
+  __syncthreads();
+  if (warp == 0) {
+    int l = 0, k = 0;
+    for (int b0 = 0; b0 < B; b0 += 32) {
+      const int b = b0 + lane;
+      const int s4 = b < B ? sb[b] & ~3 : 0, lv = b < B ? T - s4 : 0;
+      int il = lv, ik = s4;
+#pragma unroll
+      for (int o = 1; o < 32; o <<= 1) {
+        const int ul = __shfl_up_sync(0xffffffffu, il, o), uk = __shfl_up_sync(0xffffffffu, ik, o);
+        if (lane >= o) {
+          il += ul;
+          ik += uk;
+        }
+      }
+      if (b < B) {
+        live0[b] = l + il - lv;
+        skip0[b] = k + ik - s4;
+        sb[b] = s4;
+      }
+      l += __shfl_sync(0xffffffffu, il, 31);
+      k += __shfl_sync(0xffffffffu, ik, 31);
+    }
+    if (lane == 0) sched[0] = l / 4;
+  }
+  __syncthreads();
+  const int gl = (int)((N - (long)skip0[B - 1] - sb[B - 1]) / 4);
+  const int tg = T / 4;
+  for (int b = warp; b < B; b += nw) {
+    const int s4 = sb[b] / 4;
+    for (int j = lane; j < tg; j += 32) {
+      const int dst = j >= s4 ? live0[b] / 4 + (j - s4) : gl + skip0[b] / 4 + j;
+      sched[1 + dst] = b * tg + j;
+    }
+  }
+}
+
+__device__ __forceinline__ long ru_phys(const int* __restrict__ gmap, long c) {
+  return gmap ? 4L * gmap[c >> 2] + (c & 3) : c;
+}
+
+__device__ __forceinline__ void ru_tile_load_map(float* __restrict__ tile, const float* __restrict__ base,
+                                                 const int* __restrict__ gmap, long row0, long vrows, int H) {
+  if (!gmap) return ru_tile_load_async(tile, base + row0 * H, vrows * H, RU_ROWS * H);
+  const int lane = threadIdx.x & 31, gw = 4 * H;
+  for (int g = threadIdx.x >> 5; g < RU_ROWS / 4; g += RU_ROW_THREADS / 32) {
+    const bool ok = 4L * g < vrows;
+    const float* src = ok ? base + (long)gmap[(row0 >> 2) + g] * gw : base;
+    for (int j = 4 * lane; j < gw; j += 128) ru_cp_async16(tile + g * gw + j, src + j, ok ? 16 : 0);
+  }
+  cp_async_commit();
+}
+
+__device__ __forceinline__ void ru_tile_store_map(float* __restrict__ base, const float* __restrict__ tile,
+                                                  const int* __restrict__ gmap, long row0, long vrows, int H) {
+  if (!gmap) return ru_tile_store(base + row0 * H, tile, vrows * H);
+  const int lane = threadIdx.x & 31, gw = 4 * H;
+  for (int g = threadIdx.x >> 5; 4L * g < vrows; g += RU_ROW_THREADS / 32) {
+    float* dst = base + (long)gmap[(row0 >> 2) + g] * gw;
+    for (int j = 4 * lane; j < gw; j += 128)
+      *reinterpret_cast<float4*>(dst + j) = *reinterpret_cast<const float4*>(tile + g * gw + j);
+  }
+}
+
+__device__ __forceinline__ void ru_skip_share(const int* __restrict__ sched, long N, int& g0, int& g1) {
+  const int gc = sched[0], ns = (int)(N / 4) - gc, per = (ns + (int)gridDim.x - 1) / (int)gridDim.x;
+  g0 = gc + (int)blockIdx.x * per;
+  g1 = g0 + per < gc + ns ? g0 + per : gc + ns;
+  if (g0 > g1) g0 = g1;
+}
+
+template <int NT>
+__device__ __forceinline__ void ru_fill_skipped(const int* __restrict__ sched, long N, int H, float* const (&dst)[NT],
+                                                const float* const (&val)[NT], float eps, float* __restrict__ mean,
+                                                float* __restrict__ rstd, float* __restrict__ kmask,
+                                                float* __restrict__ qmask, float qflag) {
+  int g0, g1;
+  ru_skip_share(sched, N, g0, g1);
+  const int* gmap = sched + 1;
+  const int lane = threadIdx.x & 31, gw = 4 * H;
+  for (int g = g0 + (int)(threadIdx.x >> 5); g < g1; g += RU_ROW_THREADS / 32) {
+    const long off = (long)gmap[g] * gw;
+    for (int j = 4 * lane; j < gw; j += 128) {
+      int c[4];
+      c[0] = j;
+      while (c[0] >= H) c[0] -= H;
+#pragma unroll
+      for (int e = 1; e < 4; ++e) c[e] = c[e - 1] + 1 < H ? c[e - 1] + 1 : 0;
+#pragma unroll
+      for (int k = 0; k < NT; ++k) {
+        const float* v = val[k];
+        *reinterpret_cast<float4*>(dst[k] + off + j) =
+            v ? make_float4(v[c[0]], v[c[1]], v[c[2]], v[c[3]]) : make_float4(0.f, 0.f, 0.f, 0.f);
+      }
+    }
+  }
+  const float rs0 = 1.0f / sqrtf(0.f / (float)H + eps);
+  for (int i = threadIdx.x; i < 4 * (g1 - g0); i += RU_ROW_THREADS) {
+    const long row = 4L * gmap[g0 + (i >> 2)] + (i & 3);
+    mean[row] = 0.f;
+    rstd[row] = rs0;
+    if (kmask) kmask[row] = 0.f;
+    if (qmask) qmask[row] = qflag;
+  }
+}
+
 struct RuLn {
   float mean, rstd, xsum;
 };
@@ -263,6 +382,7 @@
   float *qn, *Q, *K, *V, *mean, *rstd, *kmask, *qmask;
   long N, rpc;
   int H;
+  const int* sched;
 };
 
 __global__ void __launch_bounds__(RU_THREADS, 1) ru_ln_qkv_fwd_kernel(RuLnQkvArgs a) {
@@ -302,7 +422,9 @@
   __syncthreads();
   umma::fence_after_sync();
   const uint32_t tmem = tmem_slot;
-  const RuRange rg = ru_range(a.N, a.rpc);
+  const int* gmap = a.sched ? a.sched + 1 : nullptr;
+  const long nrows = a.sched ? 4L * a.sched[0] : a.N;
+  const RuRange rg = ru_range(nrows, a.sched ? ((nrows + gridDim.x - 1) / gridDim.x + 3) / 4 * 4 : a.rpc);
   const uint32_t idesc_q = umma::idesc_tf32(128, s.NP), idesc_kv = umma::idesc_tf32(128, 2 * s.NP);
 
   if (warp == RU_ROW_THREADS / 32) {
@@ -328,17 +450,28 @@
     }
     __syncwarp();
   } else {
-    const int ntot = RU_ROWS * H;
     auto rows_of = [&](int it) {
       const long left = rg.hi - (rg.lo + (long)it * RU_ROWS);
       return left < RU_ROWS ? left : (long)RU_ROWS;
     };
     cast_pdl_wait();
-    if (rg.ntiles > 0) ru_tile_load_async(tin, a.x + rg.lo * H, rows_of(0) * H, ntot);
+    if (rg.ntiles > 0) ru_tile_load_map(tin, a.x, gmap, rg.lo, rows_of(0), H);
+    if (a.sched) {
+      float p[4];
+      for (int q = 0; q < 4; ++q) {
+        const float* y = vec + 64 + 16 * q;
+        p[q] = 0.f;
+        for (int i = 0; i < 16; i += 4) p[q] += (y[i] + y[i + 1]) + (y[i + 2] + y[i + 3]);
+      }
+      const float qflag = ((p[0] + p[1]) + (p[2] + p[3])) != 0.f ? 1.f : 0.f;
+      float* const dst[4] = {a.qn, a.K, a.V, a.Q};
+      const float* const val[4] = {vec + 64, vec + 3 * 64, vec + 4 * 64, nullptr};
+      ru_fill_skipped<4>(a.sched, a.N, H, dst, val, a.eps, a.mean, a.rstd, a.kmask, a.qmask, qflag);
+    }
     const uint32_t lane_base = ((uint32_t)(warp & 3) * 32u) << 16;
     for (int it = 0; it < rg.ntiles; ++it) {
-      const long row0 = rg.lo + (long)it * RU_ROWS, row = row0 + r;
-      const long vrows = rows_of(it), nvalid = vrows * H;
+      const long row0 = rg.lo + (long)it * RU_ROWS, rc = row0 + r;
+      const long vrows = rows_of(it);
       const uint32_t par = (uint32_t)(it & 1);
       cp_async_wait<0>();
       ru_row_sync();
@@ -349,7 +482,7 @@
       ru_operand_ready(&bars[1]);
       RU_STAMP(it, 2);
       const RuLn ln = ru_layernorm(x, q, vec, vec + 64, a.eps, r, qd, c0, H, red, [&]() {
-        if (it + 1 < rg.ntiles) ru_tile_load_async(tin, a.x + (row0 + RU_ROWS) * H, rows_of(it + 1) * H, ntot);
+        if (it + 1 < rg.ntiles) ru_tile_load_map(tin, a.x, gmap, row0 + RU_ROWS, rows_of(it + 1), H);
       });
       RU_STAMP(it, 3);
       ru_row_store(out0, r, c0, H, q);
@@ -360,7 +493,8 @@
       ru_operand_ready(&bars[2]);
       ru_row_sync();
       RU_STAMP(it, 5);
-      if (qd == 0 && row < rg.hi) {
+      if (qd == 0 && rc < rg.hi) {
+        const long row = ru_phys(gmap, rc);
         const float4 p = *reinterpret_cast<const float4*>(red + 1024 + r * 4);
         const float ysum = (p.x + p.y) + (p.z + p.w);
         a.mean[row] = ln.mean;
@@ -368,7 +502,7 @@
         if (a.kmask) a.kmask[row] = ln.xsum != 0.f ? 1.f : 0.f;
         if (a.qmask) a.qmask[row] = ysum != 0.f ? 1.f : 0.f;
       }
-      ru_tile_store(a.qn + row0 * H, out0, nvalid);
+      ru_tile_store_map(a.qn, out0, gmap, row0, vrows, H);
       float v[16];
       if (have_cols) {
         umma::tmem_ld16(tmem + lane_base + (uint32_t)(s.NP + c0), v);
@@ -378,7 +512,7 @@
       }
       ru_row_sync();
       RU_STAMP(it, 6);
-      ru_tile_store(a.K + row0 * H, out1, nvalid);
+      ru_tile_store_map(a.K, out1, gmap, row0, vrows, H);
       if (have_cols) {
         umma::tmem_ld16(tmem + lane_base + (uint32_t)(2 * s.NP + c0), v);
 #pragma unroll
@@ -387,7 +521,7 @@
       }
       ru_row_sync();
       RU_STAMP(it, 7);
-      ru_tile_store(a.V + row0 * H, out0, nvalid);
+      ru_tile_store_map(a.V, out0, gmap, row0, vrows, H);
       ru_wait(&bars[4], par);
       umma::fence_after_sync();
       RU_STAMP(it, 8);
@@ -399,7 +533,7 @@
       }
       umma::fence_before_sync();
       ru_row_sync();
-      ru_tile_store(a.Q + row0 * H, out1, nvalid);
+      ru_tile_store_map(a.Q, out1, gmap, row0, vrows, H);
       RU_STAMP(it, 9);
     }
     cp_async_wait<0>();
@@ -420,6 +554,7 @@
   float *zn, *h1d, *xout, *mean, *rstd;
   long N, rpc;
   int H;
+  const int* sched;
 };
 
 __global__ void __launch_bounds__(RU_THREADS, 1) ru_ln_ffn_fwd_kernel(RuLnFfnArgs a) {
@@ -459,7 +594,9 @@
   __syncthreads();
   umma::fence_after_sync();
   const uint32_t tmem = tmem_slot;
-  const RuRange rg = ru_range(a.N, a.rpc);
+  const int* gmap = a.sched ? a.sched + 1 : nullptr;
+  const long nrows = a.sched ? 4L * a.sched[0] : a.N;
+  const RuRange rg = ru_range(nrows, a.sched ? ((nrows + gridDim.x - 1) / gridDim.x + 3) / 4 * 4 : a.rpc);
   const uint32_t idesc = umma::idesc_tf32(128, s.NP);
   const uint32_t wpitch = (uint32_t)(s.NP * 16 + 16);
 
@@ -485,45 +622,50 @@
     }
     __syncwarp();
   } else {
-    const int ntot = RU_ROWS * H;
     auto rows_of = [&](int it) {
       const long left = rg.hi - (rg.lo + (long)it * RU_ROWS);
       return left < RU_ROWS ? left : (long)RU_ROWS;
     };
     cast_pdl_wait();
-    if (rg.ntiles > 0) ru_tile_load_async(tin, a.y + rg.lo * H, rows_of(0) * H, ntot);
+    if (rg.ntiles > 0) ru_tile_load_map(tin, a.y, gmap, rg.lo, rows_of(0), H);
+    if (a.sched) {
+      float* const dst[3] = {a.zn, a.h1d, a.xout};
+      const float* const val[3] = {nullptr, nullptr, nullptr};
+      ru_fill_skipped<3>(a.sched, a.N, H, dst, val, a.eps, a.mean, a.rstd, nullptr, nullptr, 0.f);
+    }
     const uint32_t lane_base = ((uint32_t)(warp & 3) * 32u) << 16;
     const Drop dh = make_drop(a.rate, a.seed, a.step, a.site_h);
     const Drop dout = make_drop(a.rate, a.seed, a.step, a.site_o);
     for (int it = 0; it < rg.ntiles; ++it) {
-      const long row0 = rg.lo + (long)it * RU_ROWS, row = row0 + r;
-      const long vrows = rows_of(it), nvalid = vrows * H;
+      const long row0 = rg.lo + (long)it * RU_ROWS, rc = row0 + r;
+      const long vrows = rows_of(it);
       const uint32_t par = (uint32_t)(it & 1);
-      const float m = (row < rg.hi && a.ids) ? (a.ids[row] != 0 ? 1.f : 0.f) : 1.f;
+      const float m = (rc < rg.hi && a.ids) ? (a.ids[ru_phys(gmap, rc)] != 0 ? 1.f : 0.f) : 1.f;
       cp_async_wait<0>();
       ru_row_sync();
       RU_STAMP(it, 1);
       float x[16], zn[16];
       ru_row_load(tin, r, c0, H, x);
       const RuLn ln = ru_layernorm(x, zn, vec, vec + 64, a.eps, r, qd, c0, H, red, [&]() {
-        if (it + 1 < rg.ntiles) ru_tile_load_async(tin, a.y + (row0 + RU_ROWS) * H, rows_of(it + 1) * H, ntot);
+        if (it + 1 < rg.ntiles) ru_tile_load_map(tin, a.y, gmap, row0 + RU_ROWS, rows_of(it + 1), H);
       });
       RU_STAMP(it, 2);
       ru_stage(a_hi, a_lo, r, qd, s.SL, zn);
       ru_operand_ready(&bars[1]);
       ru_row_store(out0, r, c0, H, zn);
-      if (qd == 0 && row < rg.hi) {
+      if (qd == 0 && rc < rg.hi) {
+        const long row = ru_phys(gmap, rc);
         a.mean[row] = ln.mean;
         a.rstd[row] = ln.rstd;
       }
       ru_row_sync();
       RU_STAMP(it, 3);
-      ru_tile_store(a.zn + row0 * H, out0, nvalid);
+      ru_tile_store_map(a.zn, out0, gmap, row0, vrows, H);
       ru_wait(&bars[3], par);
       umma::fence_after_sync();
       RU_STAMP(it, 4);
       float v[16];
-      const unsigned long long fi0 = (unsigned long long)(row * H + c0);
+      const unsigned long long fi0 = (unsigned long long)((rc < rg.hi ? ru_phys(gmap, rc) : rc) * H + c0);
       const bool fi_even = (fi0 & 1ull) == 0ull;
       if (have_cols) {
         umma::tmem_ld16(tmem + lane_base + (uint32_t)c0, v);
@@ -549,7 +691,7 @@
       ru_operand_ready(&bars[2]);
       ru_row_sync();
       RU_STAMP(it, 5);
-      ru_tile_store(a.h1d + row0 * H, out1, nvalid);
+      ru_tile_store_map(a.h1d, out1, gmap, row0, vrows, H);
       ru_wait(&bars[4], par);
       umma::fence_after_sync();
       RU_STAMP(it, 6);
@@ -569,7 +711,7 @@
       }
       umma::fence_before_sync();
       ru_row_sync();
-      ru_tile_store(a.xout + row0 * H, out0, nvalid);
+      ru_tile_store_map(a.xout, out0, gmap, row0, vrows, H);
       RU_STAMP(it, 7);
     }
     cp_async_wait<0>();
@@ -640,19 +782,46 @@
   return check_launch("rowk_presplit");
 }
 
+static bool ru_sched_ok(long N, std::initializer_list<const void*> ps) {
+  if (N % 4) return false;
+  for (const void* p : ps)
+    if (reinterpret_cast<uintptr_t>(p) & 15) return false;
+  return true;
+}
+
+extern "C" int cast_row_map(const int* ids, int B, int T, int* sched, void* stream) {
+  if (!ids || !sched || B <= 0 || T <= 0) return set_error(CAST_ERR_BAD_ARG, "row_map");
+  if (T % 4) return set_error(CAST_ERR_UNSUPPORTED, "row_map: maxlen must be a multiple of 4");
+  const size_t smem = 3 * (size_t)B * sizeof(int);
+  if (smem > RU_SMEM_MAX) return set_error(CAST_ERR_UNSUPPORTED, "row_map: batch too large");
+  CAST_RU_SMEM(ru_row_map_kernel, smem)
+  CAST_LAUNCH(ru_row_map_kernel, dim3(1), dim3(1024), smem, (cudaStream_t)stream, ids, B, T, sched);
+  return check_launch("row_map");
+}
+
 extern "C" int cast_rowk_ln_qkv_fwd(const float* x, const float* gamma, const float* beta, const float* bq,
                                     const float* bk, const float* bv, const void* images, long N, int H, float eps,
                                     float* qn, float* Q, float* K, float* V, float* mean, float* rstd, float* kmask,
                                     float* qmask, void* stream) {
+  return cast_rowk_ln_qkv_fwd_sched(x, gamma, beta, bq, bk, bv, images, N, H, eps, qn, Q, K, V, mean, rstd, kmask, qmask,
+                                    nullptr, stream);
+}
+
+extern "C" int cast_rowk_ln_qkv_fwd_sched(const float* x, const float* gamma, const float* beta, const float* bq,
+                                          const float* bk, const float* bv, const void* images, long N, int H, float eps,
+                                          float* qn, float* Q, float* K, float* V, float* mean, float* rstd,
+                                          float* kmask, float* qmask, const int* sched, void* stream) {
   if (!x || !gamma || !beta || !bq || !bk || !bv || !images || !qn || !Q || !K || !V || !mean || !rstd || N <= 0)
     return set_error(CAST_ERR_BAD_ARG, "rowk_ln_qkv_fwd");
+  if (sched && !ru_sched_ok(N, {x, qn, Q, K, V}))
+    return set_error(CAST_ERR_BAD_ARG, "rowk_ln_qkv_fwd: a schedule needs N % 4 == 0 and 16-byte aligned rows");
   if (!cast_rowk_supported(H)) return set_error(CAST_ERR_UNSUPPORTED, "rowk_ln_qkv_fwd: hidden_units not supported");
   const RuShape s = ru_shape(H);
   const long ntiles = cdiv(N, RU_ROWS);
   const int grid = (int)(ntiles < g_rowk_max_ctas ? ntiles : g_rowk_max_ctas);
   const long rpc = cdiv(cdiv(N, grid), 4) * 4;
   RuLnQkvArgs a{x, gamma, beta, bq, bk, bv, static_cast<const unsigned char*>(images), eps, qn, Q, K, V, mean, rstd,
-                kmask, qmask, N, rpc, H};
+                kmask, qmask, N, rpc, H, sched};
   const size_t smem = ru_ln_qkv_smem(s);
   CAST_RU_SMEM(ru_ln_qkv_fwd_kernel, smem)
   CAST_LAUNCH_DEP(ru_ln_qkv_fwd_kernel, dim3(grid), dim3(RU_THREADS), smem, (cudaStream_t)stream, a);
@@ -664,8 +833,19 @@
                                     unsigned long long seed, const unsigned long long* step, int site_hidden,
                                     int site_out, long N, int H, float eps, float* zn, float* h1d, float* xout,
                                     float* mean, float* rstd, void* stream) {
+  return cast_rowk_ln_ffn_fwd_sched(y, gamma, beta, b1, b2, images, ids, drop_rate, seed, step, site_hidden, site_out, N,
+                                    H, eps, zn, h1d, xout, mean, rstd, nullptr, stream);
+}
+
+extern "C" int cast_rowk_ln_ffn_fwd_sched(const float* y, const float* gamma, const float* beta, const float* b1,
+                                          const float* b2, const void* images, const int* ids, float drop_rate,
+                                          unsigned long long seed, const unsigned long long* step, int site_hidden,
+                                          int site_out, long N, int H, float eps, float* zn, float* h1d, float* xout,
+                                          float* mean, float* rstd, const int* sched, void* stream) {
   if (!y || !gamma || !beta || !b1 || !b2 || !images || !zn || !h1d || !xout || !mean || !rstd || N <= 0)
     return set_error(CAST_ERR_BAD_ARG, "rowk_ln_ffn_fwd");
+  if (sched && !ru_sched_ok(N, {y, zn, h1d, xout}))
+    return set_error(CAST_ERR_BAD_ARG, "rowk_ln_ffn_fwd: a schedule needs N % 4 == 0 and 16-byte aligned rows");
   if (!cast_rowk_supported(H)) return set_error(CAST_ERR_UNSUPPORTED, "rowk_ln_ffn_fwd: hidden_units not supported");
   if (drop_rate < 0.f || drop_rate >= 1.f) return set_error(CAST_ERR_BAD_ARG, "rowk_ln_ffn_fwd: drop_rate");
   const RuShape s = ru_shape(H);
@@ -673,7 +853,7 @@
   const int grid = (int)(ntiles < g_rowk_max_ctas ? ntiles : g_rowk_max_ctas);
   const long rpc = cdiv(cdiv(N, grid), 4) * 4;
   RuLnFfnArgs a{y, gamma, beta, b1, b2, static_cast<const unsigned char*>(images), ids, eps, drop_rate, seed, step,
-                site_hidden, site_out, zn, h1d, xout, mean, rstd, N, rpc, H};
+                site_hidden, site_out, zn, h1d, xout, mean, rstd, N, rpc, H, sched};
   const size_t smem = ru_ln_ffn_smem(s);
   CAST_RU_SMEM(ru_ln_ffn_fwd_kernel, smem)
   CAST_LAUNCH_DEP(ru_ln_ffn_fwd_kernel, dim3(grid), dim3(RU_THREADS), smem, (cudaStream_t)stream, a);
diff --git a/context-aware-sequential-recommendation_b200/engine.py b/context-aware-sequential-recommendation_b200/engine.py
--- a/context-aware-sequential-recommendation_b200/engine.py
+++ b/context-aware-sequential-recommendation_b200/engine.py
@@ -184,6 +184,7 @@
             self.lib.cast_set_pdl(0 if os.environ.get("CAST_PDL", "1") == "0" else 1)
         self.fork_reduce = os.environ.get("CAST_FORK_REDUCE", "1") != "0"
         self.fuse_embed_bwd = os.environ.get("CAST_FUSE_EMBED_BWD", "1") != "0"
+        self.skip_pad = os.environ.get("CAST_SKIP_PAD", "1") != "0"
         self.before_backward = None
         self.peer_adam = None
         self.shard_ptrs = None
@@ -279,6 +280,8 @@
         fp = (lambda *s: self._peer_zeros(int(np.prod(s)), torch.float32).view(*s)) if self.item_shard else f
         c = SimpleNamespace(B=B, N=N)
         c.keys3 = torch.zeros(3, N, dtype=torch.int32, device=dev)
+        c.sched = torch.zeros(1 + N // 4, dtype=torch.int32, device=dev) if T % 4 == 0 else None
+        c.sched_on = False
         c.cids = torch.zeros(3, N, dtype=torch.int32, device=dev)
         c.tw = {}
         for tower, nb in self.plan.towers.items():
@@ -431,14 +434,18 @@
             torch.cuda.current_stream(self.device).wait_stream(c.side2)
             c.presplit_pending = False
         P = self.P
+        sched = c.sched if (train and c.sched_on and ids.data_ptr() == c.keys3[0].data_ptr()) else None
+        plan = self.plan
+        x_masked = plan.embed[2] and not (plan.merge and plan.merge[3] == "pre")
         for i, b in enumerate(tb.blocks):
             pre = f"{tower}.{i}."
             if rowk:
-                self._call(self.lib.cast_rowk_ln_qkv_fwd, x.data_ptr(), P[pre + "ln1.gamma"].data_ptr(),
+                sq = sched if (i > 0 or (tower == "main" and x_masked)) else None
+                self._call(self.lib.cast_rowk_ln_qkv_fwd_sched, x.data_ptr(), P[pre + "ln1.gamma"].data_ptr(),
                            P[pre + "ln1.beta"].data_ptr(), P[pre + "q.b"].data_ptr(), P[pre + "k.b"].data_ptr(),
                            P[pre + "v.b"].data_ptr(), self.rowk_image(pre), c.N, H, 1e-8, b.qn.data_ptr(),
                            b.Q.data_ptr(), b.K.data_ptr(), b.V.data_ptr(), b.mu1.data_ptr(), b.rs1.data_ptr(),
-                           b.kmask.data_ptr(), b.qmask.data_ptr(), self._stream())
+                           b.kmask.data_ptr(), b.qmask.data_ptr(), self._p(sq), self._stream())
             elif fused:
                 self._call(self.lib.cast_ln_qkv_fwd, x.data_ptr(), P[pre + "ln1.gamma"].data_ptr(),
                            P[pre + "ln1.beta"].data_ptr(), P[pre + "q.w"].data_ptr(), P[pre + "q.b"].data_ptr(),
@@ -461,11 +468,12 @@
                        self.step_ptr, block_site(tower, i, 1), ids.data_ptr(), b.y.data_ptr(), self._p(attn),
                        b.rmax.data_ptr(), b.rlinv.data_ptr(), self._stream())
             if rowk:
-                self._call(self.lib.cast_rowk_ln_ffn_fwd, b.y.data_ptr(), P[pre + "ln2.gamma"].data_ptr(),
+                self._call(self.lib.cast_rowk_ln_ffn_fwd_sched, b.y.data_ptr(), P[pre + "ln2.gamma"].data_ptr(),
                            P[pre + "ln2.beta"].data_ptr(), P[pre + "ffn1.b"].data_ptr(), P[pre + "ffn2.b"].data_ptr(),
                            self.rowk_image(pre), ids.data_ptr(), rate, self.seed, self.step_ptr,
                            block_site(tower, i, 2), block_site(tower, i, 3), c.N, H, 1e-8, b.zn.data_ptr(),
-                           b.h1d.data_ptr(), b.xout.data_ptr(), b.mu2.data_ptr(), b.rs2.data_ptr(), self._stream())
+                           b.h1d.data_ptr(), b.xout.data_ptr(), b.mu2.data_ptr(), b.rs2.data_ptr(), self._p(sched),
+                           self._stream())
             elif fused:
                 self._call(self.lib.cast_ln_ffn_fwd, b.y.data_ptr(), P[pre + "ln2.gamma"].data_ptr(),
                            P[pre + "ln2.beta"].data_ptr(), P[pre + "ffn1.w"].data_ptr(), P[pre + "ffn1.b"].data_ptr(),
@@ -623,6 +631,12 @@
         self._call(self.lib.cast_rowk_presplit, self.rowk_wptrs, len(self.rowk_block), self.H,
                    self.rowk_img.data_ptr(), self.rowk_img.numel(), stream)
 
+    def sched_usable(self, c):
+        return self.skip_pad and self.rowk_active() and c.sched is not None
+
+    def row_map(self, c, stream):
+        self._call(self.lib.cast_row_map, c.keys3[0].data_ptr(), c.B, self.T, c.sched.data_ptr(), stream)
+
     def rowk_image(self, pre: str) -> int:
         return self.rowk_img.data_ptr() + self.rowk_block[pre] * self.rowk_img_bytes
 
@@ -819,7 +833,13 @@
                 c.side2.wait_stream(main)
                 with torch.cuda.stream(c.side2):
                     self.rowk_presplit(c.side2.cuda_stream)
+                    if self.sched_usable(c):
+                        self.row_map(c, c.side2.cuda_stream)
+                        c.sched_on = True
                 c.presplit_pending = True
+        if self.sched_usable(c) and not c.sched_on:
+            self.row_map(c, self._stream())
+            c.sched_on = True
         c.reduce_jobs = []
         c.fuse_tail = self.tail_fusable()
         bb_forked = False
@@ -846,6 +866,7 @@
             self.backward(c)
         finally:
             c.fuse_tail = False
+            c.sched_on = False
             if getattr(c, "presorted", False) or getattr(c, "presplit_pending", False):
                 main = torch.cuda.current_stream(self.device)
                 if getattr(c, "presorted", False):
diff --git a/include/cast_b200.h b/include/cast_b200.h
--- a/include/cast_b200.h
+++ b/include/cast_b200.h
@@ -107,6 +107,16 @@
                          const void* images, const int* ids, float drop_rate, unsigned long long seed,
                          const unsigned long long* step, int site_hidden, int site_out, long N, int H, float eps,
                          float* zn, float* h1d, float* xout, float* mean, float* rstd, void* stream);
+int cast_row_map(const int* ids, int B, int T, int* sched, void* stream);
+int cast_rowk_ln_qkv_fwd_sched(const float* x, const float* gamma, const float* beta, const float* bq, const float* bk,
+                               const float* bv, const void* images, long N, int H, float eps, float* qn, float* Q,
+                               float* K, float* V, float* mean, float* rstd, float* kmask, float* qmask,
+                               const int* sched, void* stream);
+int cast_rowk_ln_ffn_fwd_sched(const float* y, const float* gamma, const float* beta, const float* b1, const float* b2,
+                               const void* images, const int* ids, float drop_rate, unsigned long long seed,
+                               const unsigned long long* step, int site_hidden, int site_out, long N, int H, float eps,
+                               float* zn, float* h1d, float* xout, float* mean, float* rstd, const int* sched,
+                               void* stream);
 int cast_rowk_status(int* timed_out);
 int cast_rowk_set_grid(int max_ctas);
 int cast_rowk_set_trace(void* device_buffer);
```

New measurement: 252,500, median of 6. Within noise of the previous version (-0.0%).
